# adityaX1412/Experiment-YOLO

Measured on AMD Instinct MI355X. Metric: images/sec (train) DEAL-YOLO-N 640x640 bs=64/GPU, higher is better.
Workload: dtype f16; 1 GPU; DEAL-YOLO-N (yolov8n-ASF-P2P2.yaml) train step 640x640, per-GPU batch 64, fwd+TAL/WIOU+NWD/DFL/BCE loss+bwd+SGD+EMA, BASELINE.json configs[1]; loss_mode=wiou+nwd, settle_steps=18, capture_retries=0, global_batch=64, parallelism=dp1, hipgraph=True

## Files before the change

### experiment-yolo_amd/csrc/conv_wgrad.hip

```cpp
#include <cstdio>
#include "common.h"
#include "dealyolo_hip.h"

typedef short short4v __attribute__((ext_vector_type(4)));
typedef unsigned int u32x4 __attribute__((ext_vector_type(4)));

struct WgArgs {
  const f16* x;
  const f16* dy;
  float* slabs;
  int ldx, lddy;
  int N, H, W, Ho, Wo;
  int cin_p, cout_p;
  int cin_r8, cout_r8;
  int nci_chunks;
  int tiles_x, tiles_y, ntiles;
  long npix;
  const f16* raw;
  f16* draw;
  const float* coef;
  const double* acc;
  float* dgamma;
  float* dbeta;
  int ldraw, cout;
  float count;
  DySegs xs;
  int dy_csplit;
  unsigned dy_plane;
  const f16* wt;
  f16* dx;
  int lddx, dx_acc;
  int dg_mt, dg_rows;
  DySegs dxs;
};

static __device__ __forceinline__ half8 tr_frag(const char* base0, const char* base1) {
  union {
    short4v s[2];
    half8 h;
  } u;
  u.s[0] = __builtin_amdgcn_ds_read_tr16_b64_v4i16((LDS_AS short4v*)(base0));
  u.s[1] = __builtin_amdgcn_ds_read_tr16_b64_v4i16((LDS_AS short4v*)(base1));
  return u.h;
}

static constexpr __host__ __device__ int wg_th(int ks, int stride, int nci, int mtc) {
  if (ks == 1) return (nci + mtc <= 4) ? 8 : 4;
  if (stride == 1) return (nci * mtc <= 1) ? 16 : ((nci + mtc <= 4) ? 8 : 4);
  return (nci * mtc <= 1) ? 8 : ((nci + mtc <= 4) ? 4 : 2);
}

template <int KS, int STRIDE, int NCI, int MTC, int BNF>
__global__ __launch_bounds__(256, (BNF & 8) ? 3 : ((KS == 3 && NCI * MTC >= 16) ? 1 : 2)) void conv_wgrad_kernel(const WgArgs a) {
  constexpr bool FLAT = (KS == 1);
  constexpr bool DG = (BNF & 4) != 0;
  constexpr bool NOX = (BNF & 8) != 0;
  static_assert(!NOX || DG, "the form without X exists for the fused input gradient only");
  constexpr bool BN1 = ((BNF & 3) == 1 || (BNF & 3) == 3);
  constexpr bool XSEG = ((BNF & 3) == 3);
  static_assert(!DG || (KS == 1 && BN1), "the fused input gradient exists for the 1x1 BatchNorm forms");
  constexpr int TAPS = KS * KS;
  constexpr int NCOL = NCI * TAPS;
  constexpr int CPW = (NCOL + 3) / 4;
  constexpr int TH = wg_th(KS, STRIDE, NCI, MTC), TW = 32;
  constexpr int HWX = FLAT ? TH * TW : (TW - 1) * STRIDE + KS;
  constexpr int HHX = FLAT ? 1 : (TH - 1) * STRIDE + KS;
  constexpr int PAD = KS / 2;
  constexpr int CIN_C = 16 * NCI, COUT_C = 16 * MTC;
  constexpr int PSX = (STRIDE == 2) ? CIN_C * 2 + 16 : (((CIN_C / 2 + 7) / 16) * 16 + 8) * 4;
  constexpr int PSY = (((COUT_C / 2 + 7) / 16) * 16 + 8) * 4;
  constexpr int XBYTES = NOX ? 0 : HHX * HWX * PSX, YBYTES = TH * TW * PSY;
  __shared__ __attribute__((aligned(16))) char smem[XBYTES + YBYTES];
  char* const sx = smem;
  char* const sy = smem + XBYTES;
  __shared__ __attribute__((aligned(16))) float sbn[BN1 ? 4 * COUT_C : (BNF == 2 ? 256 * 8 : 4)];
  float bsum[8] = {0.f, 0.f, 0.f, 0.f, 0.f, 0.f, 0.f, 0.f};
  (void)bsum;
  constexpr int DKS = MTC == 4 ? 2 : (MTC == 3 ? 3 : 1), DCPK = (MTC & 1) ? 16 : 32;
  constexpr int DNT = TH / 2;
  constexpr int DNC = 4 * NCI;
  constexpr int DXROW = CIN_C * 2 + 16;
  constexpr int DPPR = CIN_C / 8;
  constexpr int DPIXPASS = 64 / DPPR > 16 ? 16 : 64 / DPPR;
  constexpr int DNPASS = (16 + DPIXPASS - 1) / DPIXPASS;
  __shared__ __attribute__((aligned(16))) char sdx[DG ? 4 * 16 * DXROW : 16];

  const int tid = threadIdx.x, wave = tid >> 6, lane = tid & 63, p = lane & 15, q = lane >> 4;
  const int qq = p >> 2, pp = p & 3;
  const int co_chunk = blockIdx.y / a.nci_chunks, ci_chunk = blockIdx.y - co_chunk * a.nci_chunks;
  const int ci0 = ci_chunk * CIN_C, co0 = co_chunk * COUT_C;

  f32x4 acc[NOX ? 1 : MTC][NOX ? 1 : CPW];
  if (!NOX) {
#pragma unroll
    for (int m = 0; m < MTC; ++m)
#pragma unroll
      for (int c = 0; c < CPW; ++c) acc[NOX ? 0 : m][NOX ? 0 : c] = (f32x4){0.f, 0.f, 0.f, 0.f};
  }
  (void)acc;

  constexpr int NGX = HHX * HWX * (CIN_C / 8), NGY = TH * TW * (COUT_C / 8);
  constexpr int NPX = NOX ? 1 : (NGX + 255) / 256, NPY = (NGY + 255) / 256;
  uint4 pfx[NPX], pfy[NPY];
  uint4 pfr[BN1 ? NPY : 1];
  unsigned roff[BN1 ? NPY : 1];
  int ncur = 0, nnext = 0;
  (void)ncur; (void)nnext;
  unsigned vnext = 0, vcur = 0, ornext = 0, orcur = 0;
  (void)pfr; (void)roff; (void)vnext; (void)vcur; (void)ornext; (void)orcur;
  constexpr unsigned NEVER = 0x80000000u;
  constexpr int CPGX = CIN_C / 8, CPGY = COUT_C / 8;
  unsigned xoff[NPX], yoff[NPY];
  (void)pfx; (void)xoff;
#pragma unroll
  for (int i = 0; i < NPX; ++i) {
    const int id = tid + i * 256;
    const int pixel = id / CPGX, part = id - pixel * CPGX;
    const bool ok = !NOX && id < NGX && ci0 + part * 8 < a.cin_r8;
    const int hy = FLAT ? 0 : pixel / HWX, hx = FLAT ? pixel : pixel - hy * HWX;
    xoff[i] = ok ? (unsigned)(((hy * a.W + hx) * a.ldx + ci0 + part * 8) * 2) : NEVER;
  }
  constexpr bool XIN = XSEG && !NOX;
  const char* xb[XIN ? NPX : 1];
  int xl[XIN ? NPX : 1];
  unsigned xup = 0;
  bool any_up = false;
  if (XIN)
    for (int k = 0; k < a.xs.nseg; ++k) any_up = any_up || (a.xs.acc[k] & 2);
  (void)xb; (void)xl; (void)xup; (void)any_up;
  if (XIN) {
#pragma unroll
    for (int i = 0; i < NPX; ++i) {
      const int id = tid + i * 256;
      const int part = id % CPGX, ch = ci0 + part * 8;
      int sg = 0;
      while (sg + 1 < a.xs.nseg && ch >= a.xs.c_end[sg]) ++sg;
      const int cb = sg ? a.xs.c_end[sg - 1] : 0;
      const bool ok = id < NGX && ch < a.cin_r8;
      xb[XIN ? i : 0] = ok ? reinterpret_cast<const char*>(a.xs.ptr[sg]) + (ch - cb) * 2 : nullptr;
      xl[XIN ? i : 0] = a.xs.ld[sg] * 2;
      if (ok && (a.xs.acc[sg] & 2)) xup |= 1u << i;
    }
  }
#pragma unroll
  for (int i = 0; i < NPY; ++i) {
    const int id = tid + i * 256;
    const int pixel = id / CPGY, part = id - pixel * CPGY;
    const bool ok = id < NGY && co0 + part * 8 < a.cout_r8;
    const int ty = FLAT ? 0 : pixel / TW, tx = FLAT ? pixel : pixel - ty * TW;
    yoff[i] = ok ? (unsigned)(((ty * a.Wo + tx) * a.lddy + co0 + part * 8) * 2) : NEVER;
    if (FLAT && BN1 && a.dy_csplit && ok) {
      const int ch = co0 + part * 8;
      yoff[i] = (unsigned)((tx * a.lddy + (ch < a.dy_csplit ? ch : ch - a.dy_csplit)) * 2) + (ch < a.dy_csplit ? 0u : a.dy_plane);
    }
    if (BN1) roff[i] = ok ? (unsigned)(((ty * a.Wo + tx) * a.ldraw + co0 + part * 8) * 2) : NEVER;
  }
  if (BN1) {
    for (int c = tid; c < COUT_C; c += 256) {
      const int ch = co0 + c;
      float sc = 0.f, sh = 0.f, kb = 0.f, kc = 0.f;
// ... 24 lines not shown
  }
  half8 wf[DG ? DKS : 1][DG ? NCI : 1];
  unsigned dboff[DG ? DKS : 1];
  char* dxb = nullptr;
  unsigned dxld2 = 0;
  bool dxacc = false, dxadd = false;
  const int dpix = lane / DPPR, dpiece = lane - dpix * DPPR;
  (void)wf; (void)dboff; (void)dxb; (void)dxld2; (void)dxacc; (void)dxadd; (void)dpix; (void)dpiece;
  if (DG) {
#pragma unroll
    for (int k = 0; k < DKS; ++k) {
      dboff[DG ? k : 0] = (unsigned)((k * DCPK + ((q * 8) & (DCPK - 1))) * 2);
#pragma unroll
      for (int j = 0; j < NCI; ++j) {
        const int ch = ci0 + (p >> 2) * DNC + 4 * j + (p & 3);
        const int gw = 16 * a.dg_mt, g = ch / gw, rem = ch - g * gw;
        const int row = g * gw + ((rem % (4 * a.dg_mt)) >> 2) * 16 + (rem / (4 * a.dg_mt)) * 4 + (rem & 3);
        const int grow = (g * DKS + k) * gw + (row - g * gw);
        half8 v;
#pragma unroll
        for (int e = 0; e < 8; ++e) v[e] = (f16)0.f;
        if (row < a.dg_rows) v = *reinterpret_cast<const half8*>(a.wt + ((size_t)grow * 32 + q * 8));
        wf[DG ? k : 0][DG ? j : 0] = v;
      }
    }
    const int chn = ci0 + dpiece * 8;
    if (lane < DPIXPASS * DPPR && chn < a.cin_r8) {
      if (XSEG) {
        int sg = 0;
        while (sg + 1 < a.dxs.nseg && chn >= a.dxs.c_end[sg]) ++sg;
        const int cb = sg ? a.dxs.c_end[sg - 1] : 0;
        dxb = reinterpret_cast<char*>(const_cast<void*>(a.dxs.ptr[sg])) + (chn - cb) * 2;
        dxld2 = (unsigned)a.dxs.ld[sg] * 2u;
        dxacc = a.dxs.acc[sg] != 0;
      } else {
        dxb = reinterpret_cast<char*>(a.dx) + chn * 2;
        dxld2 = (unsigned)a.lddx * 2u;
        dxacc = a.dx_acc != 0;
      }
    }
    if (XSEG) {
      for (int k = 0; k < a.dxs.nseg; ++k) dxadd = dxadd || a.dxs.acc[k] != 0;
    } else {
      dxadd = a.dx_acc != 0;
    }
  }
  union DU4 { uint4 u; half2_ h[4]; };
  DU4 dold[DG ? DNT : 1][DG ? DNPASS : 1];
  (void)dold;
  auto ld16 = [](__amdgpu_buffer_rsrc_t r, unsigned off) {
    const auto v = __builtin_amdgcn_raw_buffer_load_b128(r, (int)off, 0, 0);
    return *reinterpret_cast<const uint4*>(&v);
  };
  auto prefetch = [&](int tile) {
    if (FLAT) {
      const auto rx = __builtin_amdgcn_make_buffer_rsrc(const_cast<f16*>(a.x), 0, (int)((unsigned)a.npix * (unsigned)a.ldx * 2u), 0x00020000);
      const auto ry = __builtin_amdgcn_make_buffer_rsrc(const_cast<f16*>(a.dy), 0, (int)((unsigned)a.npix * (unsigned)a.lddy * 2u + (a.dy_csplit ? a.dy_plane : 0u)), 0x00020000);
      const unsigned ox = (unsigned)tile * (TH * TW) * a.ldx * 2u, oy = (unsigned)tile * (TH * TW) * a.lddy * 2u;
      if (NOX) {
      } else if (XIN) {
        const long p0 = (long)tile * (TH * TW);
        int n0 = 0, y0 = 0, x0 = 0;
        if (any_up) {
          const int hw = a.H * a.W, g0 = (int)p0;
          n0 = g0 / hw;
          const int r0 = g0 - n0 * hw;
          y0 = r0 / a.W;
          x0 = r0 - y0 * a.W;
        }
        const float invW = 1.0f / (float)a.W, invH = 1.0f / (float)a.H;
#pragma unroll
        for (int i = 0; i < NPX; ++i) {
          const int lp = (tid + i * 256) / CPGX;
          long gp = p0 + lp;
          const bool inside = gp < a.npix;
          if ((xup >> i) & 1u) {
            const int xx = x0 + lp, dy_ = (int)(((float)xx + 0.5f) * invW), x = xx - dy_ * a.W;
            const int yt = y0 + dy_, dn = (int)(((float)yt + 0.5f) * invH), y = yt - dn * a.H;
            gp = ((long)(n0 + dn) * (a.H >> 1) + (y >> 1)) * (a.W >> 1) + (x >> 1);
          }
          const char* src = xb[XIN ? i : 0];
          pfx[i] = (src && inside) ? *reinterpret_cast<const uint4*>(src + gp * xl[XIN ? i : 0]) : make_uint4(0, 0, 0, 0);
        }
      } else {
#pragma unroll
        for (int i = 0; i < NPX; ++i) pfx[i] = ld16(rx, xoff[i] + ox);
      }
#pragma unroll
      for (int i = 0; i < NPY; ++i) pfy[i] = ld16(ry, yoff[i] + oy);
      if (BN1) {
        const unsigned nbytes = (unsigned)a.npix * (unsigned)a.ldraw * 2u;
        const auto rr = __builtin_amdgcn_make_buffer_rsrc(const_cast<f16*>(a.raw), 0, (int)nbytes, 0x00020000);
        ornext = (unsigned)tile * (TH * TW) * a.ldraw * 2u;
        vnext = 0;
#pragma unroll
        for (int i = 0; i < NPY; ++i) {
          const unsigned off = roff[i] + ornext;
          pfr[i] = ld16(rr, off);
          vnext |= (roff[i] != NEVER && off < nbytes) ? (1u << i) : 0u;
        }
      }
    } else {
      const int bx = tile % a.tiles_x;
      const int t2 = tile / a.tiles_x;
      const int n = t2 / a.tiles_y;
      const int oy0 = (t2 % a.tiles_y) * TH, ox0 = bx * TW;
      const int iy0 = oy0 * STRIDE - PAD, ix0 = ox0 * STRIDE - PAD;
      const auto rx = __builtin_amdgcn_make_buffer_rsrc(const_cast<f16*>(a.x) + (size_t)n * a.H * a.W * a.ldx, 0, a.H * a.W * a.ldx * 2, 0x00020000);
      const auto ry = __builtin_amdgcn_make_buffer_rsrc(const_cast<f16*>(a.dy) + (size_t)n * a.Ho * a.Wo * a.lddy, 0, a.Ho * a.Wo * a.lddy * 2, 0x00020000);
      const unsigned ox = (unsigned)((iy0 * a.W + ix0) * a.ldx * 2), oy = (unsigned)((oy0 * a.Wo + ox0) * a.lddy * 2);
      if (ix0 >= 0 && ix0 + HWX <= a.W) {
#pragma unroll
        for (int i = 0; i < NPX; ++i) pfx[i] = ld16(rx, xoff[i] + ox);
      } else {
#pragma unroll
        for (int i = 0; i < NPX; ++i) {
          const int hx = ((tid + i * 256) / CPGX) % HWX;
          pfx[i] = ld16(rx, (unsigned)(ix0 + hx) < (unsigned)a.W ? xoff[i] + ox : NEVER);
        }
      }
      if (ox0 + TW <= a.Wo) {
#pragma unroll
        for (int i = 0; i < NPY; ++i) pfy[i] = ld16(ry, yoff[i] + oy);
      } else {
#pragma unroll
        for (int i = 0; i < NPY; ++i) {
          const int tx = ((tid + i * 256) / CPGY) % TW;
          pfy[i] = ld16(ry, ox0 + tx < a.Wo ? yoff[i] + oy : NEVER);
        }
      }
      if (BN1) {
        const unsigned nbytes = (unsigned)(a.Ho * a.Wo * a.ldraw * 2);
        const auto rr = __builtin_amdgcn_make_buffer_rsrc(const_cast<f16*>(a.raw) + (size_t)n * a.Ho * a.Wo * a.ldraw, 0, (int)nbytes, 0x00020000);
        ornext = (unsigned)((oy0 * a.Wo + ox0) * a.ldraw * 2);
        vnext = 0;
        const bool xfull = ox0 + TW <= a.Wo;
#pragma unroll
        for (int i = 0; i < NPY; ++i) {
          unsigned off = roff[i] == NEVER ? NEVER : roff[i] + ornext;
          if (!xfull) {
            const int tx = ((tid + i * 256) / CPGY) % TW;
            off = ox0 + tx < a.Wo ? off : NEVER;
          }
          pfr[i] = ld16(rr, off);
          vnext |= off < nbytes ? (1u << i) : 0u;
        }
        nnext = n;
      }
    }
  };


  int tile = (!FLAT && !(gridDim.x & 7)) ? (int)(blockIdx.x & 7) * (int)(gridDim.x >> 3) + (int)(blockIdx.x >> 3) : (int)blockIdx.x;
  if (tile < a.ntiles) prefetch(tile);
  for (; tile < a.ntiles; tile += gridDim.x) {
    __syncthreads();
#pragma unroll
    for (int i = 0; i < NPX; ++i) {
      const int id = tid + i * 256;
      if (!NOX && id < NGX) *reinterpret_cast<uint4*>(sx + (id / (CIN_C / 8)) * PSX + (id % (CIN_C / 8)) * 16) = pfx[i];
    }
    if (BN1) {
      vcur = vnext; orcur = ornext; ncur = nnext;
      const unsigned nbytes = FLAT ? (unsigned)a.npix * (unsigned)a.ldraw * 2u : (unsigned)(a.Ho * a.Wo * a.ldraw * 2);
      const auto rd = __builtin_amdgcn_make_buffer_rsrc(FLAT ? a.draw : a.draw + (size_t)ncur * a.Ho * a.Wo * a.ldraw, 0, (int)nbytes, 0x00020000);
#pragma unroll
      for (int i = 0; i < NPY; ++i) {
        const int id = tid + i * 256;
        const int part = id % CPGY;
        const bool valid = (vcur >> i) & 1u;
        const float* cf = sbn + part * 8;
        union { half8 h; uint4 u; u32x4 v; } o;
        o.h = bn_bwd_apply8<DY_ACT_SILU>(*reinterpret_cast<const half8*>(&pfy[i]), *reinterpret_cast<const half8*>(&pfr[i]), cf,
                                         cf + COUT_C, cf + 2 * COUT_C, cf + 3 * COUT_C);
        if (!valid) o.u = make_uint4(0, 0, 0, 0);
        if (id < NGY) *reinterpret_cast<uint4*>(sy + (id / (COUT_C / 8)) * PSY + (id % (COUT_C / 8)) * 16) = o.u;
        if (!DG && ci_chunk == 0 && a.draw) __builtin_amdgcn_raw_buffer_store_b128(o.v, rd, (int)(valid ? roff[i] + orcur : NEVER), 0, 0);
      }
    } else {
#pragma unroll
      for (int i = 0; i < NPY; ++i) {
        const int id = tid + i * 256;
        if (id < NGY) *reinterpret_cast<uint4*>(sy + (id / (COUT_C / 8)) * PSY + (id % (COUT_C / 8)) * 16) = pfy[i];
        if (BNF == 2 && id < NGY) {
          const half8 v = *reinterpret_cast<const half8*>(&pfy[i]);
#pragma unroll
          for (int j = 0; j < 8; ++j) bsum[j] += (float)v[j];
        }
      }
    }
    __syncthreads();
    const long dpix0 = (long)tile * (TH * TW) + wave * (16 * DNT);
    (void)dpix0;
    if (DG && dxadd) {
#pragma unroll
      for (int t = 0; t < DNT; ++t)
#pragma unroll
        for (int ps = 0; ps < DNPASS; ++ps) {
          const int rowi = ps * DPIXPASS + dpix;
          const long gp = dpix0 + t * 16 + rowi;
          const bool ok = dxb && dxacc && rowi < 16 && gp < a.npix;
          dold[DG ? t : 0][DG ? ps : 0].u = ok ? *reinterpret_cast<const uint4*>(dxb + (size_t)gp * dxld2) : make_uint4(0, 0, 0, 0);
        }
      __builtin_amdgcn_sched_barrier(0);
    }
    if (tile + (int)gridDim.x < a.ntiles) prefetch(tile + gridDim.x);
// ... 193 lines not shown
    const int mid = (lo + hi + 1) >> 1;
    if (descs[mid].first_block <= (int)blockIdx.x) lo = mid;
    else hi = mid - 1;
  }
  const WgReduceDesc d = descs[lo];
  if (d.bias_c > 0 && (int)blockIdx.x == d.first_block && (int)threadIdx.x < d.bias_c) {
    double t = 0.0;
#pragma unroll
    for (int k = 0; k < DY_BN_COPIES; ++k) t += d.bias_acc[(size_t)k * d.bias_c + threadIdx.x];
    d.dbias[threadIdx.x] = (float)t;
  }
  wgrad_reduce_block(blockIdx.x - d.first_block, d.slabs, d.nslabs, d.dw, d.cout, d.cin, d.taps, d.cout_p, d.cin_p, d.accumulate,
                     d.ld_taps, d.ld_cphys, d.ld_cin);
}
extern "C" int dy_wgrad_reduce_desc_bytes(void) { return (int)sizeof(WgReduceDesc); }
static void wgrad_geometry(int cin, int cout, int ks, int stride, int* cin_p, int* cout_p, int* nci, int* mtc, long npix_out = 0);
extern "C" int dy_wgrad_reduce_desc_fill(void* desc, const float* slabs, int nslabs, float* dw, int cin, int cout, int ks, int stride,
                                         int accumulate, int ld_taps, int ld_cphys, int ld_cin, int first_block) {
  if (!desc || !slabs || !dw || nslabs < 1) return DY_ERR_ARG;
  int cp, op, nci, mtc;
  const int cin_eff = ld_taps ? ld_taps * ld_cphys : cin;
  wgrad_geometry(cin_eff, cout, ld_taps ? 1 : ks, ld_taps ? 1 : stride, &cp, &op, &nci, &mtc);
  const int taps = ld_taps ? 1 : ks * ks;
  WgReduceDesc* d = reinterpret_cast<WgReduceDesc*>(desc);
  *d = WgReduceDesc{slabs, dw, nslabs, cout, cin_eff, taps, op, cp, accumulate, ld_taps, ld_cphys, ld_cin, first_block, 0, nullptr, nullptr};
  return cdiv(taps * op * cp, 64);
}
extern "C" int dy_wgrad_reduce_desc_bias(void* desc, const double* bias_acc, float* dbias, int c) {
  if (!desc || !bias_acc || !dbias || c < 1 || c > 256) return DY_ERR_ARG;
  WgReduceDesc* d = reinterpret_cast<WgReduceDesc*>(desc);
  d->bias_acc = bias_acc; d->dbias = dbias; d->bias_c = c;
  return DY_OK;
}
extern "C" int dy_wgrad_reduce_batched(const void* descs_device, int n, int total_blocks, hipStream_t stream) {
  if (n <= 0 || total_blocks <= 0 || !descs_device) return DY_ERR_ARG;
  hipLaunchKernelGGL(wgrad_reduce_batched_kernel, dim3(total_blocks), dim3(256), 0, stream, (const WgReduceDesc*)descs_device, n);
  DY_CHECK_LAUNCH();
  return DY_OK;
}

template <int KS, int STRIDE, int NCI, int MTC>
static int launch_wgrad(const WgArgs& a, int gx, int gy, hipStream_t s) {
  if (a.wt) {
    if constexpr (KS == 1) {
      if (!a.raw || gy != a.nci_chunks) return DY_ERR_ARG;
      if (!a.x) {
        if (a.dxs.nseg > 0) hipLaunchKernelGGL((conv_wgrad_kernel<KS, STRIDE, NCI, MTC, 15>), dim3(gx, gy), dim3(256), 0, s, a);
        else hipLaunchKernelGGL((conv_wgrad_kernel<KS, STRIDE, NCI, MTC, 13>), dim3(gx, gy), dim3(256), 0, s, a);
      } else if (a.xs.nseg > 0) hipLaunchKernelGGL((conv_wgrad_kernel<KS, STRIDE, NCI, MTC, 7>), dim3(gx, gy), dim3(256), 0, s, a);
      else hipLaunchKernelGGL((conv_wgrad_kernel<KS, STRIDE, NCI, MTC, 5>), dim3(gx, gy), dim3(256), 0, s, a);
    } else return DY_ERR_ARG;
  } else if (a.raw && a.xs.nseg > 0) {
    if constexpr (KS == 1) hipLaunchKernelGGL((conv_wgrad_kernel<KS, STRIDE, NCI, MTC, 3>), dim3(gx, gy), dim3(256), 0, s, a);
    else return DY_ERR_ARG;
  } else if (a.raw) hipLaunchKernelGGL((conv_wgrad_kernel<KS, STRIDE, NCI, MTC, 1>), dim3(gx, gy), dim3(256), 0, s, a);
  else if (a.acc && MTC != 3) hipLaunchKernelGGL((conv_wgrad_kernel<KS, STRIDE, NCI, MTC, 2>), dim3(gx, gy), dim3(256), 0, s, a);
  else if (a.acc) return DY_ERR_ARG;
  else hipLaunchKernelGGL((conv_wgrad_kernel<KS, STRIDE, NCI, MTC, 0>), dim3(gx, gy), dim3(256), 0, s, a);
  DY_CHECK_LAUNCH();
  return DY_OK;
}
template <int KS, int STRIDE>
static int dispatch_wgrad(int nci, int mtc, const WgArgs& a, int gx, int gy, hipStream_t s) {
#define DY_CASE(I, M) \
  if (nci == I && mtc == M) return launch_wgrad<KS, STRIDE, I, M>(a, gx, gy, s);
  DY_CASE(1, 1) DY_CASE(1, 2) DY_CASE(1, 4)
  DY_CASE(2, 1) DY_CASE(2, 2) DY_CASE(2, 4)
  if (!(KS == 3 && STRIDE == 2)) { DY_CASE(4, 1) DY_CASE(4, 2) DY_CASE(4, 4) }
  if (KS == 1) {
    DY_CASE(3, 1) DY_CASE(3, 2) DY_CASE(3, 4) DY_CASE(1, 3) DY_CASE(2, 3) DY_CASE(4, 3) DY_CASE(3, 3)
  }
#undef DY_CASE
  return DY_ERR_ARG;
}

static int wgrad_per_cu(int ks, int nci, int mtc) {
  static const int light = getenv("DY_WGRAD_LIGHT_WGS") ? atoi(getenv("DY_WGRAD_LIGHT_WGS")) : 2;
  if (ks == 3 && nci * mtc >= 16) return 1;
  return nci * mtc <= 2 ? light : 2;
}
static long wgrad_columns(int ks, int nci, int mtc, int cp, int op) {
  const int gy = (cp / (16 * nci)) * (op / (16 * mtc));
  const int per_cu = wgrad_per_cu(ks, nci, mtc);
  int gx = (256 * per_cu) / gy;
  return gx < 32 ? 32 : gx;
}
static void wgrad_geometry(int cin, int cout, int ks, int stride, int* cin_p, int* cout_p, int* nci, int* mtc, long npix_out) {
  *cin_p = (cin + 15) / 16 * 16;
  *cout_p = (cout + 15) / 16 * 16;
  const int cit = *cin_p / 16, cot = *cout_p / 16;
  const int cap = (ks == 3 && stride == 2) ? 2 : 4;
  *nci = (cit % 4 == 0 && cap >= 4) ? 4 : ((ks == 1 && cit % 3 == 0) ? 3 : (cit % 2 == 0 ? 2 : 1));
  *mtc = cot % 4 == 0 ? 4 : ((ks == 1 && cot % 3 == 0) ? 3 : (cot % 2 == 0 ? 2 : 1));
  static const bool split = !(getenv("DY_WGRAD_SPLIT") && atoi(getenv("DY_WGRAD_SPLIT")) == 0);
  static const double f = getenv("DY_WGRAD_SPLIT_F") ? atof(getenv("DY_WGRAD_SPLIT_F")) : 2.0;
  if (!split || npix_out <= 0) return;
  const double wbytes = (double)ks * ks * *cin_p * *cout_p * 4.0;
  const double act = (double)npix_out * (*cin_p * stride * stride + *cout_p) * 2.0;
  while (2.0 * wgrad_columns(ks, *nci, *mtc, *cin_p, *cout_p) * wbytes > f * act) {
    if (*mtc % 2 == 0 && *mtc >= *nci) *mtc /= 2;
    else if (*nci % 2 == 0) *nci /= 2;
    else if (*mtc % 2 == 0) *mtc /= 2;
    else break;
  }
}

extern "C" int dy_wgrad_workspace(int n, int h, int w, int cin, int cout, int ks, int stride, int* nslabs,
                                  long* slab_elems) {
  int cp, op, nci, mtc;
  const int pad = ks / 2, Ho = (h + 2 * pad - ks) / stride + 1, Wo = (w + 2 * pad - ks) / stride + 1;
  wgrad_geometry(cin, cout, ks, stride, &cp, &op, &nci, &mtc, (long)n * Ho * Wo);
  const int th = wg_th(ks, stride, nci, mtc);
  int ntiles;
  if (ks == 1) ntiles = (int)(((long)n * Ho * Wo + th * 32 - 1) / (th * 32));
  else ntiles = cdiv(Wo, 32) * cdiv(Ho, th) * n;
  *slab_elems = (long)ks * ks * cp * op;
  const int gy = (cp / (16 * nci)) * (op / (16 * mtc));
  const int per_cu = wgrad_per_cu(ks, nci, mtc);
  int gx = (256 * per_cu) / gy;
  if (gx < 32) gx = 32;
  static const int tpb = getenv("DY_WGRAD_TPB") ? atoi(getenv("DY_WGRAD_TPB")) : 1;
  if (tpb > 1 && gx > ntiles / tpb) gx = ntiles / tpb > 32 ? ntiles / tpb : (ntiles < 32 ? ntiles : 32);
  if (gx > ntiles) gx = ntiles;
  if (gx < 1) gx = 1;
  *nslabs = gx;
  return DY_OK;
}

struct WgBnHost {
  const void* raw; void* draw; const float* coef; const double* acc; float* dgamma; float* dbeta; int ldraw; float count;
  const DySegs* xs = nullptr;
  int dy_csplit = 0;
  unsigned dy_plane = 0;
  const void* wt = nullptr; void* dx = nullptr; int lddx = 0, dx_acc = 0; const DySegs* dxs = nullptr;
  bool dgrad_only = false;
};
static int conv_wgrad_impl(const void* x, int ldx, const void* dy, int lddy, float* slabs, float* dw, int n, int h, int w,
                           int cin, int cout, int ks, int stride, int accumulate, int ld_taps, int ld_cphys, int ld_cin,
                           hipStream_t stream, const WgBnHost* bn = nullptr);

extern "C" int dy_wgrad_kernel_name(int cin, int cout, int ks, int stride, char* out, int cap) {
  if (!out || cap < 8) return DY_ERR_ARG;
  int cp, op, nci, mtc;
  wgrad_geometry(cin, cout, ks, stride, &cp, &op, &nci, &mtc);
  snprintf(out, cap, "conv_wgrad_kernel<%d, %d, %d, %d, 0>", ks, stride, nci, mtc);
  return DY_OK;
}

extern "C" int dy_wgrad_kernel_name_at(int n, int h, int w, int cin, int cout, int ks, int stride, char* out, int cap) {
  if (!out || cap < 8) return DY_ERR_ARG;
  int cp, op, nci, mtc;
  wgrad_geometry(cin, cout, ks, stride, &cp, &op, &nci, &mtc,
                 (long)n * ((h + 2 * (ks / 2) - ks) / stride + 1) * ((w + 2 * (ks / 2) - ks) / stride + 1));
  snprintf(out, cap, "conv_wgrad_kernel<%d, %d, %d, %d, 0>", ks, stride, nci, mtc);
  return DY_OK;
}

extern "C" int dy_conv_wgrad(const void* x, int ldx, const void* dy, int lddy, float* slabs, float* dw, int n, int h,
                             int w, int cin, int cout, int ks, int stride, int accumulate, hipStream_t stream) {
  return conv_wgrad_impl(x, ldx, dy, lddy, slabs, dw, n, h, w, cin, cout, ks, stride, accumulate, 0, 0, 0, stream);
}
extern "C" int dy_conv_wgrad_ld(const void* x, int ldx, const void* dy, int lddy, float* slabs, float* dw, int n, int h,
                                int w, int cout, int ld_cin, int ld_taps, int ld_cphys, int accumulate, hipStream_t stream) {
  return conv_wgrad_impl(x, ldx, dy, lddy, slabs, dw, n, h, w, ld_taps * ld_cphys, cout, 1, 1, accumulate, ld_taps, ld_cphys,
                         ld_cin, stream);
}

extern "C" int dy_conv_wgrad_bn(const void* x, int ldx, const void* dy, int lddy, const void* raw, int ldraw, void* draw,
                                const float* coef, const double* acc, float* dgamma, float* dbeta, float count, float* slabs,
                                float* dw, int n, int h, int w, int cin, int cout, int ks, int stride, int accumulate,
                                hipStream_t stream) {
  if (!raw || !coef || !acc || (ldraw & 7) || ((uintptr_t)raw & 15) || ((uintptr_t)draw & 15) || (cout & 15)) return DY_ERR_ARG;
  const WgBnHost bn{raw, draw, coef, acc, dgamma, dbeta, ldraw, count};
  return conv_wgrad_impl(x, ldx, dy, lddy, slabs, dw, n, h, w, cin, cout, ks, stride, accumulate, 0, 0, 0, stream, &bn);
}
extern "C" int dy_conv_wgrad_bias(const void* x, int ldx, const void* dy, int lddy, double* bias_acc, float* slabs, float* dw, int n,
                                  int h, int w, int cin, int cout, int ks, int stride, int accumulate, hipStream_t stream) {
  if (!bias_acc) return DY_ERR_ARG;
  const WgBnHost bn{nullptr, nullptr, nullptr, bias_acc, nullptr, nullptr, 0, 1.f};
  return conv_wgrad_impl(x, ldx, dy, lddy, slabs, dw, n, h, w, cin, cout, ks, stride, accumulate, 0, 0, 0, stream, &bn);
}
extern "C" int dy_conv1x1_wgrad_bn_segs(const DySegs* xs, const void* dy, int lddy, const void* raw, int ldraw, void* draw, const float* coef,
                                        const double* acc, float* dgamma, float* dbeta, float count, float* slabs, float* dw, int n, int h,
                                        int w, int cin, int cout, int accumulate, hipStream_t stream) {
  if (!raw || !coef || !acc || (ldraw & 7) || ((uintptr_t)raw & 15) || ((uintptr_t)draw & 15) || (cout & 15)) return DY_ERR_ARG;
  if (!xs || xs->nseg < 1 || xs->nseg > DY_MAX_SEGS || xs->c_end[xs->nseg - 1] != cin) return DY_ERR_ARG;
  for (int k = 0; k < xs->nseg; ++k)
    if ((xs->c_end[k] & 7) || (xs->ld[k] & 7) || !xs->ptr[k] || ((uintptr_t)xs->ptr[k] & 15) || xs->c_end[k] <= (k ? xs->c_end[k - 1] : 0) ||
        ((xs->acc[k] & 2) && ((h | w) & 1))) return DY_ERR_ARG;
  WgBnHost bn{raw, draw, coef, acc, dgamma, dbeta, ldraw, count};
  bn.xs = xs;
  return conv_wgrad_impl(xs->ptr[0], 8, dy, lddy, slabs, dw, n, h, w, cin, cout, 1, 1, accumulate, 0, 0, 0, stream, &bn);
}
extern "C" int dy_conv1x1_wgrad_bn_planes(const DySegs* xs, const void* x, int ldx, const void* dy, const void* dy2, int lddy, int csplit,
                                          const void* raw, int ldraw, void* draw, const float* coef, const double* acc, float* dgamma,
                                          float* dbeta, float count, float* slabs, float* dw, int n, int h, int w, int cin, int cout,
                                          int accumulate, hipStream_t stream) {
  if (!raw || !coef || !acc || (ldraw & 7) || ((uintptr_t)raw & 15) || ((uintptr_t)draw & 15) || (cout & 15)) return DY_ERR_ARG;
  if (!dy || !dy2 || (csplit & 7) || csplit <= 0 || csplit >= cout || ((uintptr_t)dy2 & 15)) return DY_ERR_ARG;
  const long plane = (const char*)dy2 - (const char*)dy;
  if (plane < (long)n * h * w * lddy * 2 || plane + (double)n * h * w * lddy * 2.0 >= 2147483648.0) return DY_ERR_ARG;
  if (xs) {
    if (xs->nseg < 1 || xs->nseg > DY_MAX_SEGS || xs->c_end[xs->nseg - 1] != cin) return DY_ERR_ARG;
    for (int k = 0; k < xs->nseg; ++k)
      if ((xs->c_end[k] & 7) || (xs->ld[k] & 7) || !xs->ptr[k] || ((uintptr_t)xs->ptr[k] & 15) || xs->c_end[k] <= (k ? xs->c_end[k - 1] : 0) ||
          ((xs->acc[k] & 2) && ((h | w) & 1))) return DY_ERR_ARG;
  }
  WgBnHost bn{raw, draw, coef, acc, dgamma, dbeta, ldraw, count};
  bn.xs = xs;
  bn.dy_csplit = csplit; bn.dy_plane = (unsigned)plane;
  return conv_wgrad_impl(xs ? xs->ptr[0] : x, xs ? 8 : ldx, dy, lddy, slabs, dw, n, h, w, cin, cout, 1, 1, accumulate, 0, 0, 0, stream, &bn);
}

struct WgDgPlan { int ok, nci, mtc, dg_mt, dg_rows; };
static WgDgPlan wgrad_dgrad_plan(int n, int h, int w, int cin, int cout) {
  WgDgPlan r{};
  if (n < 1 || h < 1 || w < 1 || cin < 8 || (cin & 7) || cout < 16 || (cout & 15) || cout > 64) return r;
  int cp, op, nci, mtc;
  wgrad_geometry(cin, cout, 1, 1, &cp, &op, &nci, &mtc, (long)n * h * w);
  if (16 * mtc != op) return r;
  int gcin, gcout, cc, nch, mt, ng, kst, pe;
  if (dy_conv_geometry(cout, cin, 1, 1, &gcin, &gcout, &cc, &nch, &mt, &ng, &kst, &pe) != DY_OK) return r;
  const int dks = mtc == 4 ? 2 : (mtc == 3 ? 3 : 1), dcpk = (mtc & 1) ? 16 : 32;
  if (gcin != cout || nch * kst != dks || (cc < 32 ? cc : 32) != dcpk || gcout < cp) return r;
  r.ok = 1; r.nci = nci; r.mtc = mtc; r.dg_mt = mt; r.dg_rows = gcout;
  return r;
// ... 91 lines not shown
                                                int lddx, int dx_accumulate, const DySegs* dxs, int n, int h, int w, int cin, int cout,
                                                int accumulate, hipStream_t stream) {
  if (!raw || !coef || !acc || (ldraw & 7) || ((uintptr_t)raw & 15)) return DY_ERR_ARG;
  if (!dy || !dy2 || (csplit & 7) || csplit <= 0 || csplit >= cout || ((uintptr_t)dy2 & 15)) return DY_ERR_ARG;
  const long plane = (const char*)dy2 - (const char*)dy;
  if (plane < (long)n * h * w * lddy * 2 || plane + (double)n * h * w * lddy * 2.0 >= 2147483648.0) return DY_ERR_ARG;
  if (!w_packed_t || ((uintptr_t)w_packed_t & 15) || !wgrad_dgrad_plan(n, h, w, cin, cout).ok) return DY_ERR_ARG;
  if (xs) {
    if (!segs_in_valid(xs, cin, h, w) || !dgrad_segs_valid(xs, dxs)) return DY_ERR_ARG;
  } else if (dxs || !dx || ((uintptr_t)dx & 15) || (lddx & 7) || lddx < cin || (double)n * h * w * lddx * 2.0 >= 2147483648.0) {
    return DY_ERR_ARG;
  }
  WgBnHost bn{raw, nullptr, coef, acc, dgamma, dbeta, ldraw, count};
  bn.xs = xs; bn.dy_csplit = csplit; bn.dy_plane = (unsigned)plane;
  bn.wt = w_packed_t; bn.dxs = xs ? dxs : nullptr; bn.dx = xs ? nullptr : dx; bn.lddx = lddx; bn.dx_acc = dx_accumulate != 0;
  return conv_wgrad_impl(xs ? xs->ptr[0] : x, xs ? 8 : ldx, dy, lddy, slabs, dw, n, h, w, cin, cout, 1, 1, accumulate, 0, 0, 0, stream, &bn);
}
extern "C" int dy_conv_wgrad_ld_bn(const void* x, int ldx, const void* dy, int lddy, const void* raw, int ldraw, void* draw,
                                   const float* coef, const double* acc, float* dgamma, float* dbeta, float count, float* slabs,
                                   float* dw, int n, int h, int w, int cout, int ld_cin, int ld_taps, int ld_cphys, int accumulate,
                                   hipStream_t stream) {
  if (!raw || !coef || !acc || (ldraw & 7) || ((uintptr_t)raw & 15) || ((uintptr_t)draw & 15) || (cout & 15)) return DY_ERR_ARG;
  const WgBnHost bn{raw, draw, coef, acc, dgamma, dbeta, ldraw, count};
  return conv_wgrad_impl(x, ldx, dy, lddy, slabs, dw, n, h, w, ld_taps * ld_cphys, cout, 1, 1, accumulate, ld_taps, ld_cphys, ld_cin,
                         stream, &bn);
}

static int conv_wgrad_impl(const void* x, int ldx, const void* dy, int lddy, float* slabs, float* dw, int n, int h, int w,
                           int cin, int cout, int ks, int stride, int accumulate, int ld_taps, int ld_cphys, int ld_cin,
                           hipStream_t stream, const WgBnHost* bn) {
  if (!(ks == 1 || ks == 3) || !(stride == 1 || stride == 2) || (ks == 1 && stride != 1)) return DY_ERR_ARG;
  if ((ldx & 7) || (lddy & 7) || ((uintptr_t)x & 15) || ((uintptr_t)dy & 15)) return DY_ERR_ALIGN;
  const bool dgrad_only = bn && bn->dgrad_only;
  if (dgrad_only != (x == nullptr) || (dgrad_only && (!bn->wt || slabs || dw))) return DY_ERR_ARG;
  if ((ks == 1 ? (double)n : 1.0) * h * w * (ldx > lddy ? ldx : lddy) * 2.0 >= 2147483648.0) return DY_ERR_ARG;
  int cp, op, nci, mtc;
  wgrad_geometry(cin, cout, ks, stride, &cp, &op, &nci, &mtc,
                 (long)n * ((h + 2 * (ks / 2) - ks) / stride + 1) * ((w + 2 * (ks / 2) - ks) / stride + 1));
  WgArgs a{};
  a.x = (const f16*)x; a.dy = (const f16*)dy; a.slabs = slabs; a.ldx = ldx; a.lddy = lddy;
  a.N = n; a.H = h; a.W = w;
  const int pad = ks / 2;
  a.Ho = (h + 2 * pad - ks) / stride + 1;
  a.Wo = (w + 2 * pad - ks) / stride + 1;
  a.cin_p = cp; a.cout_p = op;
  a.cin_r8 = (cin + 7) / 8 * 8; a.cout_r8 = (cout + 7) / 8 * 8;
  if (bn) {
    if ((ks == 1 ? (double)n : 1.0) * a.Ho * a.Wo * bn->ldraw * 2.0 >= 2147483648.0) return DY_ERR_ARG;
    a.raw = (const f16*)bn->raw; a.draw = (f16*)bn->draw; a.coef = bn->coef; a.acc = bn->acc;
    a.dgamma = bn->dgamma; a.dbeta = bn->dbeta; a.ldraw = bn->ldraw; a.count = bn->count;
    a.cout = bn->raw ? cout : (cout + 7) / 8 * 8;
    if (bn->xs) a.xs = *bn->xs;
    a.dy_csplit = bn->dy_csplit; a.dy_plane = bn->dy_plane;
    if (bn->wt) {
      const WgDgPlan pl = wgrad_dgrad_plan(n, h, w, cin, cout);
      if (!pl.ok || pl.nci != nci || pl.mtc != mtc || ks != 1 || ld_taps) return DY_ERR_ARG;
      a.wt = (const f16*)bn->wt; a.dx = (f16*)bn->dx; a.lddx = bn->lddx; a.dx_acc = bn->dx_acc;
      a.dg_mt = pl.dg_mt; a.dg_rows = pl.dg_rows;
      if (bn->dxs) a.dxs = *bn->dxs;
    }
  }
  a.nci_chunks = cp / (16 * nci);
  const int nco_chunks = op / (16 * mtc);
  const int th = wg_th(ks, stride, nci, mtc);
  if (ks == 1) {
    a.npix = (long)n * a.Ho * a.Wo;
    a.ntiles = (int)((a.npix + th * 32 - 1) / (th * 32));
  } else {
    a.tiles_x = cdiv(a.Wo, 32);
    a.tiles_y = cdiv(a.Ho, th);
    a.ntiles = a.tiles_x * a.tiles_y * n;
  }
  int nslabs;
  long slab_elems;
  dy_wgrad_workspace(n, h, w, cin, cout, ks, stride, &nslabs, &slab_elems);
  const int gy = a.nci_chunks * nco_chunks;
  if (dgrad_only) nslabs = dgrad_only_columns(a.ntiles, gy);
  int rc;
  if (ks == 1) rc = dispatch_wgrad<1, 1>(nci, mtc, a, nslabs, gy, stream);
  else if (stride == 1) rc = dispatch_wgrad<3, 1>(nci, mtc, a, nslabs, gy, stream);
  else rc = dispatch_wgrad<3, 2>(nci, mtc, a, nslabs, gy, stream);
  if (rc != DY_OK) return rc;
  if (!dw) return DY_OK;
  const int total = ks * ks * op * cp;
  hipLaunchKernelGGL(wgrad_reduce_kernel, dim3(cdiv(total, 64)), dim3(256), 0, stream, slabs, nslabs, dw, cout, cin,
                     ks * ks, op, cp, accumulate, ld_taps, ld_cphys, ld_cin);
  DY_CHECK_LAUNCH();
  return DY_OK;
}
```

### experiment-yolo_amd/csrc/head_rows.hip

```cpp
#include <hip/hip_runtime.h>

#include <cstdlib>

#include "common.h"
#include "dealyolo_hip.h"

template <typename T>
struct Levels {
  int nl;
  T lv[4];
};
struct RowsArgs {
  const f16* x;
  const f16* dy;
  const int* flag;
  const float* w;
  f16* dx;
  float* slabs;
  double* bias_acc;
  int ldx, lddy, lddx, A, a0, hw, B, dx_acc;
  const float* xcoef;
  int nblk, dgx;
};

// ... 25 lines not shown
          fl[k] = a.flag[(size_t)b * a.A + a.a0 + r];
        }
      }
    }
    int mine = -1;
#pragma unroll
    for (int k = 0; k < FB; ++k)
      if ((trip & (FB - 1)) == k) mine = fl[k];
    const bool fg = mine >= 0;
    const unsigned long long m = __ballot(fg);
    if (lane == 0) s_cnt[wave] = __popcll(m);
    __syncthreads();
    int base = 0, total = 0;
#pragma unroll
    for (int w = 0; w < 4; ++w) {
      if (w < wave) base += s_cnt[w];
      total += s_cnt[w];
    }
    if (fg) s_list[base + __popcll(m & ((1ull << lane) - 1ull))] = tid;
    __syncthreads();
    for (int i0 = 0; i0 < total; i0 += 16) {
      const int nb = total - i0 < 16 ? total - i0 : 16;
      {
        const int i = tid >> 4, g = tid & 15;
        if (i < nb) {
          const long q = p0 + s_list[i0 + i];
          if (g < 8) {
            half8 xv = *reinterpret_cast<const half8*>(a.x + q * a.ldx + g * 8);
            if (a.xcoef) xv = bn_silu_apply8(xv, a.xcoef + g * 8, a.xcoef + 64 + g * 8);
            *reinterpret_cast<half8*>(s_x + i * 64 + g * 8) = xv;
          } else {
            *reinterpret_cast<uint4*>(s_dy + i * 64 + (g - 8) * 8) = *reinterpret_cast<const uint4*>(a.dy + q * a.lddy + (g - 8) * 8);
          }
        }
      }
      __syncthreads();
      for (int i = 0; i < nb; ++i) {
        const float g = (float)s_dy[i * 64 + co];
#pragma unroll
        for (int k = 0; k < 16; ++k) acc[k] += g * (float)s_x[i * 64 + ci0 + k];
        if ((tid & 3) == 0) bs += g;
      }
      __syncthreads();
    }
  }
  float* slab = a.slabs + (size_t)blockIdx.x * 64 * 64 + co * 64 + ci0;
#pragma unroll
  for (int k = 0; k < 16; k += 4) *reinterpret_cast<float4*>(slab + k) = make_float4(acc[k], acc[k + 1], acc[k + 2], acc[k + 3]);
  if ((tid & 3) == 0 && bs != 0.f) unsafeAtomicAdd(a.bias_acc + (size_t)(blockIdx.x % DY_BN_COPIES) * 64 + co, (double)bs);
}

__global__ __launch_bounds__(256) void rows_dgrad_kernel(Levels<RowsArgs> L) {
  const RowsArgs& a = L.lv[blockIdx.z];
  if (!a.dx || (int)blockIdx.x >= a.dgx || (int)blockIdx.y >= a.B) return;
  __shared__ float s_w[64 * 65];
  for (int i = threadIdx.x; i < 64 * 64; i += 256) s_w[(i >> 6) * 65 + (i & 63)] = (float)(f16)a.w[i];
  __syncthreads();
  const int b = blockIdx.y, part = threadIdx.x & 7, ci0 = part * 8;
  const int* const fl = a.flag + (size_t)b * a.A + a.a0;
  for (int r = (int)(blockIdx.x * 32 + (threadIdx.x >> 3)); r < a.hw; r += a.dgx * 32) {
    const long p = (long)b * a.hw + r;
    f16* const dst = a.dx + p * a.lddx + ci0;
    if (fl[r] < 0) {
      if (!a.dx_acc) *reinterpret_cast<uint4*>(dst) = make_uint4(0, 0, 0, 0);
      continue;
    }
    float s[8];
#pragma unroll
    for (int k = 0; k < 8; ++k) s[k] = 0.f;
    const f16* const g = a.dy + p * a.lddy;
    for (int c8 = 0; c8 < 64; c8 += 8) {
      const half8 gv = *reinterpret_cast<const half8*>(g + c8);
#pragma unroll
      for (int j = 0; j < 8; ++j) {
        const float gg = (float)gv[j];
#pragma unroll
        for (int k = 0; k < 8; ++k) s[k] += gg * s_w[(c8 + j) * 65 + ci0 + k];
      }
    }
    half8 o;
    if (a.dx_acc) {
      const half8 old = *reinterpret_cast<const half8*>(dst);
#pragma unroll
      for (int k = 0; k < 8; ++k) o[k] = (f16)((float)old[k] + s[k]);
    } else {
#pragma unroll
      for (int k = 0; k < 8; ++k) o[k] = (f16)s[k];
    }
    *reinterpret_cast<half8*>(dst) = o;
  }
}

static __device__ __forceinline__ float exp_nonpos(float x) {
  const float t = x * 1.44269502f;
  float r = __builtin_fmaf(x, 1.44269502f, -t);
  r = __builtin_fmaf(x, 1.92596299e-8f, r);
  const float e = __builtin_amdgcn_exp2f(t);
  return __builtin_fmaf(e, r * 0.693147182f, e);
}
static __device__ __forceinline__ f32x2 exp_nonpos2(f32x2 x) {
  const f32x2 l2e = {1.44269502f, 1.44269502f}, l2e_lo = {1.92596299e-8f, 1.92596299e-8f}, ln2 = {0.693147182f, 0.693147182f};
  const f32x2 t = x * l2e;
  f32x2 r = __builtin_elementwise_fma(x, l2e, -t);
  r = __builtin_elementwise_fma(x, l2e_lo, r);
  const f32x2 e = {__builtin_amdgcn_exp2f(t[0]), __builtin_amdgcn_exp2f(t[1])};
  return __builtin_elementwise_fma(e, r * ln2, e);
}
struct BoxDecArgs {
  const f16* x;
  const float* w;
  const float* bias;
  float* pred_box;
  int ldx, A, a0, hw, W, B;
  const float* xcoef;
  int nblk;
};
template <bool LIBM>
__global__ __launch_bounds__(256) void head_box_decode_kernel(Levels<BoxDecArgs> L) {
  const BoxDecArgs& a = L.lv[blockIdx.y];
  if ((int)blockIdx.x >= a.nblk) return;
  auto ex = [](float x) { return LIBM ? expf(x) : exp_nonpos(x); };
  constexpr int PITCH = 160;
  __shared__ __attribute__((aligned(16))) char s_w[64 * PITCH];
  __shared__ float s_b[64];
  const int tid = threadIdx.x, wave = tid >> 6, lane = tid & 63, p = lane & 15, q = lane >> 4;
  for (int i = tid; i < 64 * 64; i += 256) {
    const int c = i >> 6, k = i & 63;
    const int row = ((c >> 2) & 3) * 16 + (c >> 4) * 4 + (c & 3);
    *reinterpret_cast<f16*>(s_w + row * PITCH + k * 2) = (f16)a.w[i];
  }
  if (tid < 64) s_b[tid] = a.bias[tid];
  __syncthreads();
  const long npix = (long)a.B * a.hw;
  const float invw = 1.0f / (float)a.W;
  float csc[2][8], csh[2][8];
  if (a.xcoef) {
#pragma unroll
    for (int ks = 0; ks < 2; ++ks)
#pragma unroll
      for (int j = 0; j < 8; ++j) {
        csc[ks][j] = a.xcoef[ks * 32 + q * 8 + j];
        csh[ks][j] = a.xcoef[64 + ks * 32 + q * 8 + j];
// ... 62 lines not shown
      const float anc = (q & 1) ? (iy + 0.5f) : (ix + 0.5f);
      a.pred_box[((size_t)b * a.A + a.a0 + r) * 4 + q] = q < 2 ? anc - e : anc + e;
    }
  }
}
static int box_decode_fill(BoxDecArgs& a, const void* x, int ldx, const float* x_coef, const float* weight, const float* bias, float* pred_box,
                           int A, int a0, int n, int h, int w, int cin, int cout) {
  if (cin != 64 || cout != 64 || !x || !weight || !bias || !pred_box || n < 1 || h < 1 || w < 1 || a0 < 0 || a0 + h * w > A) return DY_ERR_ARG;
  if ((ldx & 7) || ((uintptr_t)x & 15)) return DY_ERR_ALIGN;
  static const int cap = getenv("DY_HEAD_DECODE_WGS") ? atoi(getenv("DY_HEAD_DECODE_WGS")) : 2048;
  long blocks = ((long)n * h * w + 255) / 256;
  if (blocks > cap) blocks = cap;
  a = BoxDecArgs{(const f16*)x, weight, bias, pred_box, ldx, A, a0, h * w, w, n, x_coef, (int)blocks};
  return DY_OK;
}
static int box_decode_launch(const Levels<BoxDecArgs>& L, hipStream_t stream) {
  int gx = 1;
  for (int l = 0; l < L.nl; ++l) gx = L.lv[l].nblk > gx ? L.lv[l].nblk : gx;
  static const bool libm = getenv("DY_DECODE_LIBM_EXP") && atoi(getenv("DY_DECODE_LIBM_EXP")) != 0;
  if (libm) hipLaunchKernelGGL(head_box_decode_kernel<true>, dim3(gx, L.nl), dim3(256), 0, stream, L);
  else hipLaunchKernelGGL(head_box_decode_kernel<false>, dim3(gx, L.nl), dim3(256), 0, stream, L);
  DY_CHECK_LAUNCH();
  return DY_OK;
}
extern "C" int dy_head_box_decode(const void* x, int ldx, const float* x_coef, const float* weight, const float* bias, float* pred_box, int A,
                                  int a0, int n, int h, int w, int cin, int cout, hipStream_t stream) {
  Levels<BoxDecArgs> L{};
  L.nl = 1;
  const int rc = box_decode_fill(L.lv[0], x, ldx, x_coef, weight, bias, pred_box, A, a0, n, h, w, cin, cout);
  return rc != DY_OK ? rc : box_decode_launch(L, stream);
}
extern "C" int dy_head_box_decode_levels(int nl, const void* const* x, const int* ldx, const float* const* x_coef, const float* const* weight,
                                         const float* const* bias, float* pred_box, int A, const int* a0, int n, const int* h, const int* w,
                                         int cin, int cout, hipStream_t stream) {
  if (nl < 1 || nl > 4) return DY_ERR_ARG;
  Levels<BoxDecArgs> L{};
  L.nl = nl;
  for (int l = 0; l < nl; ++l) {
    const int rc = box_decode_fill(L.lv[l], x[l], ldx[l], x_coef ? x_coef[l] : nullptr, weight[l], bias[l], pred_box, A, a0[l], n, h[l], w[l], cin, cout);
    if (rc != DY_OK) return rc;
  }
  return box_decode_launch(L, stream);
}

extern "C" int dy_conv1x1_rows_supported(int cin, int cout) { return cin == 64 && cout == 64; }
extern "C" int dy_conv1x1_rows_slabs(int n, int h, int w) {
  const long ns = (long)n * h * w / 2048;
  return ns < 64 ? 64 : (ns > 1024 ? 1024 : (int)ns);
}
static int rows_fill(RowsArgs& a, const void* x, int ldx, const float* x_coef, const void* dy, int lddy, const int* assigned, int A, int a0,
                     const float* weight, void* dx, int lddx, int dx_accumulate, float* slabs, double* bias_acc, int n, int h, int w, int cin,
                     int cout) {
  if (!dy_conv1x1_rows_supported(cin, cout) || !x || !dy || !assigned || !weight || !slabs || !bias_acc || n < 1 || h < 1 || w < 1 ||
      a0 < 0 || a0 + h * w > A)
    return DY_ERR_ARG;
  if ((ldx & 7) || (lddy & 7) || (dx && (lddx & 7)) || ((uintptr_t)x & 15) || ((uintptr_t)dy & 15) || ((uintptr_t)dx & 15) ||
      ((uintptr_t)slabs & 15))
    return DY_ERR_ALIGN;
  int gx = (h * w + 1023) / 1024;
  if (gx > 16) gx = 16;
  a = RowsArgs{(const f16*)x, (const f16*)dy, assigned, weight, (f16*)dx, slabs, bias_acc, ldx, lddy, lddx, A, a0, h * w, n, dx_accumulate, x_coef,
               dy_conv1x1_rows_slabs(n, h, w), gx};
  return DY_OK;
}
static int rows_launch(const Levels<RowsArgs>& L, hipStream_t stream) {
  int gw = 1, gd = 0, nb = 1;
  for (int l = 0; l < L.nl; ++l) {
    gw = L.lv[l].nblk > gw ? L.lv[l].nblk : gw;
    if (L.lv[l].dx) gd = L.lv[l].dgx > gd ? L.lv[l].dgx : gd;
    nb = L.lv[l].B > nb ? L.lv[l].B : nb;
  }
  hipLaunchKernelGGL(rows_wgrad_kernel, dim3(gw, L.nl), dim3(256), 0, stream, L);
  if (gd) hipLaunchKernelGGL(rows_dgrad_kernel, dim3(gd, nb, L.nl), dim3(256), 0, stream, L);
  DY_CHECK_LAUNCH();
  return DY_OK;
}
extern "C" int dy_conv1x1_rows_backward(const void* x, int ldx, const float* x_coef, const void* dy, int lddy, const int* assigned, int A, int a0,
                                        const float* weight, void* dx, int lddx, int dx_accumulate, float* slabs, double* bias_acc,
                                        int n, int h, int w, int cin, int cout, hipStream_t stream) {
  Levels<RowsArgs> L{};
  L.nl = 1;
  const int rc = rows_fill(L.lv[0], x, ldx, x_coef, dy, lddy, assigned, A, a0, weight, dx, lddx, dx_accumulate, slabs, bias_acc, n, h, w, cin, cout);
  return rc != DY_OK ? rc : rows_launch(L, stream);
}
extern "C" int dy_conv1x1_rows_backward_levels(int nl, const void* const* x, const int* ldx, const float* const* x_coef, const void* const* dy,
                                               const int* lddy, const int* assigned, int A, const int* a0, const float* const* weight,
                                               void* const* dx, const int* lddx, const int* dx_accumulate, float* const* slabs,
                                               double* const* bias_acc, int n, const int* h, const int* w, int cin, int cout,
                                               hipStream_t stream) {
  if (nl < 1 || nl > 4) return DY_ERR_ARG;
  Levels<RowsArgs> L{};
  L.nl = nl;
  for (int l = 0; l < nl; ++l) {
    const int rc = rows_fill(L.lv[l], x[l], ldx[l], x_coef ? x_coef[l] : nullptr, dy[l], lddy[l], assigned, A, a0[l], weight[l], dx[l], lddx[l],
                             dx_accumulate[l], slabs[l], bias_acc[l], n, h[l], w[l], cin, cout);
    if (rc != DY_OK) return rc;
  }
  return rows_launch(L, stream);
}

struct ClsArgs {
  const f16* x;
  const float* xcoef;
  const float* w;
  const float* bias;
  float* y;
  const f16* dy;
  f16* dx;
  float* slabs;
  double* bias_acc;
  int ldx, lddx, nc, dx_acc;
  long npix;
  int nblk;
};
template <int CIN>
__global__ __launch_bounds__(256) void cls_head_fwd_kernel(Levels<ClsArgs> L) {
  const ClsArgs& a = L.lv[blockIdx.y];
  if ((int)blockIdx.x >= a.nblk) return;
  constexpr int PARTS = CIN / 8, PPB = 256 / PARTS;
  __shared__ float s_w[8][CIN], s_b[8];
  for (int i = threadIdx.x; i < 8 * CIN; i += 256) s_w[i / CIN][i % CIN] = (i / CIN) < a.nc ? (float)(f16)a.w[i] : 0.f;
  if (threadIdx.x < 8) s_b[threadIdx.x] = threadIdx.x < a.nc ? a.bias[threadIdx.x] : 0.f;
  __syncthreads();
  const int part = threadIdx.x % PARTS, k0 = part * 8;
  float sc[8], sh[8];
  if (a.xcoef) {
#pragma unroll
    for (int j = 0; j < 8; ++j) { sc[j] = a.xcoef[k0 + j]; sh[j] = a.xcoef[CIN + k0 + j]; }
  }
  for (long pix = (long)blockIdx.x * PPB + threadIdx.x / PARTS; pix < a.npix; pix += (long)a.nblk * PPB) {
    half8 xv = *reinterpret_cast<const half8*>(a.x + pix * a.ldx + k0);
    if (a.xcoef) xv = bn_silu_apply8(xv, sc, sh);
    float o[8];
#pragma unroll
    for (int c = 0; c < 8; ++c) {
      float t = 0.f;
#pragma unroll
      for (int j = 0; j < 8; ++j) t += s_w[c][k0 + j] * (float)xv[j];
      o[c] = t;
    }
#pragma unroll
    for (int c = 0; c < 8; ++c) o[c] = PARTS == 4 ? quad_sum(o[c]) : half_row_sum(o[c]);
    if (part == 0) {
      float* dst = a.y + pix * 8;
      *reinterpret_cast<float4*>(dst) = make_float4(o[0] + s_b[0], o[1] + s_b[1], o[2] + s_b[2], o[3] + s_b[3]);
      *reinterpret_cast<float4*>(dst + 4) = make_float4(o[4] + s_b[4], o[5] + s_b[5], o[6] + s_b[6], o[7] + s_b[7]);
    }
  }
}
template <int CIN>
__global__ __launch_bounds__(256) void cls_head_bwd_kernel(Levels<ClsArgs> L) {
  const ClsArgs& a = L.lv[blockIdx.y];
  if ((int)blockIdx.x >= a.nblk) return;
  constexpr int PARTS = CIN / 8, PPB = 256 / PARTS;
  __shared__ float s_w[8][CIN];
  __shared__ float s_red[4][PARTS][64];
  __shared__ float s_bs[4][8];
  for (int i = threadIdx.x; i < 8 * CIN; i += 256) s_w[i / CIN][i % CIN] = (i / CIN) < a.nc ? (float)(f16)a.w[i] : 0.f;
  __syncthreads();
  const int tid = threadIdx.x, wave = tid >> 6, lane = tid & 63, part = tid % PARTS, k0 = part * 8;
  float sc[8], sh[8];
  if (a.xcoef) {
#pragma unroll
    for (int j = 0; j < 8; ++j) { sc[j] = a.xcoef[k0 + j]; sh[j] = a.xcoef[CIN + k0 + j]; }
  }
  float acc[8][8], bs[8];
#pragma unroll
  for (int c = 0; c < 8; ++c) {
    bs[c] = 0.f;
#pragma unroll
    for (int j = 0; j < 8; ++j) acc[c][j] = 0.f;
  }
  const long chunk = ((a.npix + a.nblk - 1) / a.nblk + PPB - 1) / PPB * PPB;
  const long lo = (long)blockIdx.x * chunk, hi = lo + chunk < a.npix ? lo + chunk : a.npix;
  for (long pix = lo + tid / PARTS; pix < hi; pix += PPB) {
    half8 xv = *reinterpret_cast<const half8*>(a.x + pix * a.ldx + k0);
    const half8 dv = *reinterpret_cast<const half8*>(a.dy + pix * 8);
    if (a.xcoef) xv = bn_silu_apply8(xv, sc, sh);
    float d[8], g[8];
#pragma unroll
    for (int c = 0; c < 8; ++c) d[c] = (float)dv[c];
#pragma unroll
    for (int j = 0; j < 8; ++j) g[j] = 0.f;
#pragma unroll
    for (int c = 0; c < 8; ++c) {
#pragma unroll
      for (int j = 0; j < 8; ++j) {
        acc[c][j] += d[c] * (float)xv[j];
        g[j] += s_w[c][k0 + j] * d[c];
      }
      if (part == 0) bs[c] += d[c];
    }
    if (a.dx) {
      f16* dst = a.dx + pix * a.lddx + k0;
      half8 o;
      if (a.dx_acc) {
        const half8 old = *reinterpret_cast<const half8*>(dst);
#pragma unroll
        for (int j = 0; j < 8; ++j) o[j] = (f16)((float)old[j] + g[j]);
      } else {
#pragma unroll
        for (int j = 0; j < 8; ++j) o[j] = (f16)g[j];
      }
      *reinterpret_cast<half8*>(dst) = o;
    }
  }
#pragma unroll
  for (int c = 0; c < 8; ++c) {
#pragma unroll
    for (int j = 0; j < 8; ++j) {
      float v = acc[c][j];
#pragma unroll
      for (int m = PARTS; m < 64; m <<= 1) v += __shfl_xor(v, m, 64);
      acc[c][j] = v;
    }
    float b = bs[c];
#pragma unroll
    for (int m = PARTS; m < 64; m <<= 1) b += __shfl_xor(b, m, 64);
    bs[c] = b;
  }
  if (lane < PARTS) {
#pragma unroll
    for (int c = 0; c < 8; ++c)
#pragma unroll
      for (int j = 0; j < 8; ++j) s_red[wave][lane][c * 8 + j] = acc[c][j];
  }
  if (lane == 0) {
#pragma unroll
    for (int c = 0; c < 8; ++c) s_bs[wave][c] = bs[c];
  }
  __syncthreads();
  float* slab = a.slabs + (size_t)blockIdx.x * 16 * CIN;
  for (int i = tid; i < 16 * CIN; i += 256) {
    const int co = i / CIN, ci = i - co * CIN;
    float v = 0.f;
    if (co < 8) {
      const int pp = ci >> 3, j = ci & 7;
      v = (s_red[0][pp][co * 8 + j] + s_red[1][pp][co * 8 + j]) + (s_red[2][pp][co * 8 + j] + s_red[3][pp][co * 8 + j]);
    }
    slab[i] = v;
  }
  if (tid < 8) {
    const float b = (s_bs[0][tid] + s_bs[1][tid]) + (s_bs[2][tid] + s_bs[3][tid]);
    if (b != 0.f) unsafeAtomicAdd(a.bias_acc + (size_t)(blockIdx.x % DY_BN_COPIES) * 8 + tid, (double)b);
  }
}
extern "C" int dy_cls_head_supported(int cin, int nc) { return (cin == 32 || cin == 64) && nc >= 1 && nc <= 8; }
extern "C" int dy_cls_head_slabs(void) { return 512; }
static int cls_fill(ClsArgs& a, bool backward, const void* x, int ldx, const float* x_coef, const float* weight, const float* bias, float* logits,
                    const void* dy, void* dx, int lddx, int dx_accumulate, float* slabs, double* bias_acc, long npix, int cin, int nc) {
  if (!dy_cls_head_supported(cin, nc) || !x || !weight || npix < 1) return DY_ERR_ARG;
  if (!backward && (!bias || !logits)) return DY_ERR_ARG;
  if (backward && (!dy || !slabs || !bias_acc)) return DY_ERR_ARG;
  if ((ldx & 7) || (dx && (lddx & 7)) || ((uintptr_t)x & 15) || ((uintptr_t)logits & 15) || ((uintptr_t)dy & 15) || ((uintptr_t)dx & 15))
    return DY_ERR_ALIGN;
  int nblk;
  if (backward) {
    nblk = dy_cls_head_slabs();
  } else {
    const int ppb = 256 / (cin / 8);
    long blocks = (npix + ppb - 1) / ppb;
    nblk = (int)(blocks > 4096 ? 4096 : blocks);
  }
  a = ClsArgs{(const f16*)x, x_coef, weight, bias, logits, (const f16*)dy, (f16*)dx, slabs, bias_acc, ldx, lddx, nc, dx_accumulate, npix, nblk};
  return DY_OK;
}
static int cls_launch(const Levels<ClsArgs>& L, bool backward, int cin, hipStream_t stream) {
  int gx = 1;
  for (int l = 0; l < L.nl; ++l) gx = L.lv[l].nblk > gx ? L.lv[l].nblk : gx;
  const dim3 grid(gx, L.nl);
  if (!backward && cin == 32) hipLaunchKernelGGL(cls_head_fwd_kernel<32>, grid, dim3(256), 0, stream, L);
  else if (!backward) hipLaunchKernelGGL(cls_head_fwd_kernel<64>, grid, dim3(256), 0, stream, L);
  else if (cin == 32) hipLaunchKernelGGL(cls_head_bwd_kernel<32>, grid, dim3(256), 0, stream, L);
  else hipLaunchKernelGGL(cls_head_bwd_kernel<64>, grid, dim3(256), 0, stream, L);
  DY_CHECK_LAUNCH();
  return DY_OK;
}
extern "C" int dy_cls_head_forward(const void* x, int ldx, const float* x_coef, const float* weight, const float* bias, float* logits,
                                   long npix, int cin, int nc, hipStream_t stream) {
  Levels<ClsArgs> L{};
  L.nl = 1;
  const int rc = cls_fill(L.lv[0], false, x, ldx, x_coef, weight, bias, logits, nullptr, nullptr, 0, 0, nullptr, nullptr, npix, cin, nc);
  return rc != DY_OK ? rc : cls_launch(L, false, cin, stream);
}
extern "C" int dy_cls_head_backward(const void* x, int ldx, const float* x_coef, const void* dy, const float* weight, void* dx, int lddx,
                                    int dx_accumulate, float* slabs, double* bias_acc, long npix, int cin, int nc, hipStream_t stream) {
  Levels<ClsArgs> L{};
  L.nl = 1;
  const int rc = cls_fill(L.lv[0], true, x, ldx, x_coef, weight, nullptr, nullptr, dy, dx, lddx, dx_accumulate, slabs, bias_acc, npix, cin, nc);
  return rc != DY_OK ? rc : cls_launch(L, true, cin, stream);
}
extern "C" int dy_cls_head_forward_levels(int nl, const void* const* x, const int* ldx, const float* const* x_coef, const float* const* weight,
                                          const float* const* bias, float* const* logits, const long* npix, int cin, int nc,
                                          hipStream_t stream) {
  if (nl < 1 || nl > 4) return DY_ERR_ARG;
  Levels<ClsArgs> L{};
  L.nl = nl;
  for (int l = 0; l < nl; ++l) {
    const int rc = cls_fill(L.lv[l], false, x[l], ldx[l], x_coef ? x_coef[l] : nullptr, weight[l], bias[l], logits[l], nullptr, nullptr, 0, 0, nullptr,
                            nullptr, npix[l], cin, nc);
    if (rc != DY_OK) return rc;
  }
  return cls_launch(L, false, cin, stream);
}
extern "C" int dy_cls_head_backward_levels(int nl, const void* const* x, const int* ldx, const float* const* x_coef, const void* const* dy,
                                           const float* const* weight, void* const* dx, const int* lddx, const int* dx_accumulate,
                                           float* const* slabs, double* const* bias_acc, const long* npix, int cin, int nc,
                                           hipStream_t stream) {
  if (nl < 1 || nl > 4) return DY_ERR_ARG;
  Levels<ClsArgs> L{};
  L.nl = nl;
  for (int l = 0; l < nl; ++l) {
    const int rc = cls_fill(L.lv[l], true, x[l], ldx[l], x_coef ? x_coef[l] : nullptr, weight[l], nullptr, nullptr, dy[l], dx[l], lddx[l],
                            dx_accumulate[l], slabs[l], bias_acc[l], npix[l], cin, nc);
    if (rc != DY_OK) return rc;
  }
  return cls_launch(L, true, cin, stream);
}
```

### experiment-yolo_amd/csrc/loss.hip

```cpp
#include "common.h"
#include "dealyolo_hip.h"

#define REG_MAX 16
#define TOPK 10
#define TAL_EPS 1e-9f
#define IOU_EPS 1e-7f

struct Level {
  const float* box;
  const float* cls;
  f16* dbox;
  f16* dcls;
  int H, W, a0;
  float stride;
  const f16* xin = nullptr;
  int ldin = 0;
  const float* w = nullptr;
  const float* bias = nullptr;
  const float* incoef = nullptr;
};
struct BoxMode {
  int family, ltype, fm, modifier;
  float inner_ratio, focaler_d, focaler_u, shape_scale, piou_lambda;
  float mpd_hw_num;
// ... 297 lines not shown
  const Dual cw = dmaximum(x2, dconst(t[2])) - dminimum(x1, dconst(t[0]));
  const Dual ch = dmaximum(y2, dconst(t[3])) - dminimum(y1, dconst(t[1]));
  if (m.ltype == DY_BOX_GIOU) {
    const Dual ca = cw * ch + IOU_EPS;
    return I - (ca - uni) / ca;
  }
  const Dual c2 = (dsq(cw) + dsq(ch)) + IOU_EPS;
  const Dual sx = ((t[0] + t[2]) - x1) - x2, sy = ((t[1] + t[3]) - y1) - y2;
  const Dual rho2 = (dsq(sx) + dsq(sy)) / 4.f;
  switch (m.ltype) {
    case DY_BOX_CIOU: {
      const Dual v = (float)(4.0 / (M_PI * M_PI)) * dsq(atanf(w2 / h2) - t_atan(w1 / h1));
      const float alpha = v.v / ((v.v - Ia.v) + (1.f + IOU_EPS));
      return I - (rho2 / c2 + v * alpha);
    }
    case DY_BOX_EIOU: {
      const Dual rw2 = dsq((t[2] - t[0]) - (x2 - x1)), rh2 = dsq((t[3] - t[1]) - (y2 - y1));
      return I - ((rho2 / c2 + rw2 / (dsq(cw) + IOU_EPS)) + rh2 / (dsq(ch) + IOU_EPS));
    }
    case DY_BOX_SIOU: {
      const Dual scw = sx * 0.5f + IOU_EPS, sch = sy * 0.5f + IOU_EPS;
      const Dual sigma = t_sqrt(dsq(scw) + dsq(sch));
      const Dual s1 = dabs(scw) / sigma, s2 = dabs(sch) / sigma;
      const Dual sa = dsel(s1.v > 0.70710678118654752f, s2, s1);
      const Dual gamma = dcos(dasin(sa) * 2.f - (float)(M_PI / 2)) - 2.f;
      const Dual dc = (2.f - t_exp(gamma * dsq(scw / cw))) - t_exp(gamma * dsq(sch / ch));
      const Dual ow = dabs(w1 - w2) / dmaximum(w1, dconst(w2)), oh = dabs(h1 - h2) / dmaximum(h1, dconst(h2));
      const Dual sc = dpow4(1.f - t_exp(-ow)) + dpow4(1.f - t_exp(-oh));
      return (I - 0.5f * (dc + sc)) + IOU_EPS;
    }
    case DY_BOX_SHAPEIOU: {
      const float pws = powf(w2, m.shape_scale), phs = powf(h2, m.shape_scale);
      const float ww = 2.f * pws / (pws + phs), hh = 2.f * phs / (pws + phs);
      const Dual dist = (hh * (dsq(sx) / 4.f) + ww * (dsq(sy) / 4.f)) / c2;
      const Dual ow = (hh * dabs(w1 - w2)) / dmaximum(w1, dconst(w2)), oh = (ww * dabs(h1 - h2)) / dmaximum(h1, dconst(h2));
      const Dual sc = dpow4(1.f - t_exp(-ow)) + dpow4(1.f - t_exp(-oh));
      return (I - dist) - 0.5f * sc;
    }
    case DY_BOX_PIOU:
    case DY_BOX_PIOU2: {
      const Dual dw1 = dabs(dminimum(x2, x1) - fminf(t[2], t[0])), dw2 = dabs(dmaximum(x2, x1) - fmaxf(t[2], t[0]));
      const Dual dh1 = dabs(dminimum(y2, y1) - fminf(t[3], t[1])), dh2 = dabs(dmaximum(y2, y1) - fmaxf(t[3], t[1]));
      const Dual P = ((dw1 + dw2) / fabsf(w2) + (dh1 + dh2) / fabsf(h2)) / 4.f;
      const Dual pv1 = ((1.f - I) - t_exp(-dsq(P))) + 1.f;
      if (m.ltype == DY_BOX_PIOU) return 1.f - pv1;
      const Dual x = t_exp(-P) * m.piou_lambda;
      return 1.f - ((3.f * x) * t_exp(-dsq(x))) * pv1;
    }
    default:
      return I - rho2 / c2;
  }
}

__global__ void pack_targets_kernel(LossCtx c, const float* bidx, const float* cls, const float* boxes, int n,
                                    const int* n_dev, float img_w, float img_h) {
  if (n_dev) n = *n_dev;
  for (int i = blockIdx.x * blockDim.x + threadIdx.x; i < c.B * c.nmax; i += gridDim.x * blockDim.x) {
    c.gt_valid[i] = 0;
    c.gt_cls[i] = 0;
    c.pos_align[i] = 0u;
    c.pos_ov[i] = 0u;
    for (int k = 0; k < 4; ++k) c.gt_box[i * 4 + k] = 0.f;
  }
  if (threadIdx.x == 0) c.scal[9] = 0.f;
  __shared__ short sb[8192];
  const int ncache = n < 8192 ? n : 8192;
  for (int i = threadIdx.x; i < ncache; i += blockDim.x) sb[i] = (short)(int)bidx[i];
  __syncthreads();
  for (int i = threadIdx.x; i < n; i += blockDim.x) {
    const int b = (int)bidx[i];
    if (b < 0 || b >= c.B) continue;
    int slot = 0;
    for (int j = 0; j < i; ++j) slot += ((j < ncache ? (int)sb[j] : (int)bidx[j]) == b);
    if (slot >= c.nmax) {
      c.scal[9] = 1.f;
      c.scal[10] = 1.f;
      continue;
    }
    const float x = boxes[i * 4 + 0] * img_w, y = boxes[i * 4 + 1] * img_h;
    const float w = boxes[i * 4 + 2] * img_w, h = boxes[i * 4 + 3] * img_h;
    const float dw = w / 2, dh = h / 2;
    float* g = c.gt_box + ((size_t)b * c.nmax + slot) * 4;
    g[0] = x - dw; g[1] = y - dh; g[2] = x + dw; g[3] = y + dh;
    c.gt_cls[b * c.nmax + slot] = (int)cls[i];
    c.gt_valid[b * c.nmax + slot] = (g[0] + g[1] + g[2] + g[3]) > 0.f ? 1 : 0;
  }
}

static __device__ __forceinline__ float softmax16_expect(float logit, int bin, float& prob) {
  float m = logit;
  m = fmaxf(m, __shfl_xor(m, 1, 64));
  m = fmaxf(m, __shfl_xor(m, 2, 64));
  m = fmaxf(m, __shfl_xor(m, 4, 64));
  m = fmaxf(m, __shfl_xor(m, 8, 64));
  const float e = expf(logit - m);
  const float s = quad16_sum(e);
  prob = e / s;
  return quad16_sum(prob * (float)bin);
}

__global__ __launch_bounds__(256) void decode_kernel(LossCtx c) {
  const int sub = threadIdx.x & 15, side = sub >> 2, quarter = sub & 3;
  const int b = blockIdx.y;
  float invw[4];
#pragma unroll
  for (int k = 0; k < 4; ++k) invw[k] = k < c.nl ? 1.0f / (float)c.lv[k].W : 0.f;
  for (int a = (int)((blockIdx.x * 256 + threadIdx.x) >> 4); a < c.A; a += (int)((gridDim.x * 256) >> 4)) {
    int l = 0;
#pragma unroll
    for (int k = 1; k < 4; ++k)
      if (k < c.nl && a >= c.lv[k].a0) l = k;
    const Level& L = c.lv[l];
    const int r = a - L.a0;
    const int iy = (int)(((float)r + 0.5f) * invw[l]), ix = r - iy * L.W;
    const float4 v = *reinterpret_cast<const float4*>(L.box + ((size_t)b * (L.H * L.W) + r) * 64 + sub * 4);
    float m = fmaxf(fmaxf(v.x, v.y), fmaxf(v.z, v.w));
    m = fmaxf(m, __shfl_xor(m, 1, 64));
    m = fmaxf(m, __shfl_xor(m, 2, 64));
    const float e0 = expf(v.x - m), e1 = expf(v.y - m), e2 = expf(v.z - m), e3 = expf(v.w - m);
    float den = (e0 + e1) + (e2 + e3);
    const float k0 = (float)(quarter * 4);
    float num = e0 * k0 + e1 * (k0 + 1.f) + e2 * (k0 + 2.f) + e3 * (k0 + 3.f);
    den += __shfl_xor(den, 1, 64);
    num += __shfl_xor(num, 1, 64);
    den += __shfl_xor(den, 2, 64);
    num += __shfl_xor(num, 2, 64);
// ... 514 lines not shown
  hipLaunchKernelGGL(tal_scatter_kernel, dim3(cdiv((int)BN * TOPK, 256)), dim3(256), 0, stream, c);
  const int gridE = (int)((BA + 255) / 256 < 2048 ? (BA + 255) / 256 : 2048);
  hipLaunchKernelGGL(tal_resolve_kernel, dim3(gridE), dim3(256), 0, stream, c);
  hipLaunchKernelGGL(tal_scores_kernel, dim3(gridE), dim3(256), 0, stream, c);
  DY_CHECK_LAUNCH();
  return DY_OK;
}

extern "C" int dy_loss_args_bytes(void) { return (int)sizeof(DyLossArgs); }
extern "C" int dy_detection_loss(const DyLossArgs* d, hipStream_t stream) {
  if (d->nl < 1 || d->nl > 4 || d->nmax < 1 || (d->ncp & 7) || d->nc > d->ncp) return DY_ERR_ARG;
  LossCtx c{};
  c.nl = d->nl; c.B = d->B; c.nc = d->nc; c.ncp = d->ncp; c.nmax = d->nmax;
  int a0 = 0;
  for (int l = 0; l < d->nl; ++l) {
    c.lv[l] = Level{d->box[l], d->cls[l], (f16*)d->dbox[l], (f16*)d->dcls[l], d->H[l], d->W[l], a0, d->stride[l]};
    if (d->box_from_input) {
      if (!d->box_in[l] || !d->box_w[l] || !d->box_b[l] || (d->box_in_ld[l] & 7)) return DY_ERR_ARG;
      c.lv[l].box = nullptr;
      c.lv[l].xin = (const f16*)d->box_in[l]; c.lv[l].ldin = d->box_in_ld[l]; c.lv[l].w = d->box_w[l]; c.lv[l].bias = d->box_b[l];
      c.lv[l].incoef = d->box_in_coef[l];
    }
    a0 += d->H[l] * d->W[l];
  }
  c.A = a0;
  char* p = (char*)d->workspace;
  auto take = [&](size_t b) { char* r = p; p += (b + 255) / 256 * 256; return r; };
  const size_t BA = (size_t)c.B * c.A, BN = (size_t)c.B * c.nmax;
  c.gt_box = (float*)take(BN * 16); c.gt_cls = (int*)take(BN * 4); c.gt_valid = (int*)take(BN * 4);
  c.pred_box = (float*)take(BA * 16); c.cnt = (int*)take(BA * 4); c.owner = (int*)take(BA * 4);
  c.asg_gt = (int*)take(BA * 4); c.asg_metric = (float*)take(BA * 4); c.asg_ov = (float*)take(BA * 4);
  c.tscore = (float*)take(BA * 4);
  c.topk_idx = (int*)take(BN * TOPK * 4); c.pos_align = (unsigned*)take(BN * 4); c.pos_ov = (unsigned*)take(BN * 4);
  float* scal_ws = (float*)take(16 * 4);
  (void)scal_ws;
  c.scal = d->scalars;
  float* partA = (float*)take(3 * 4096 * 4);
  float* partB = (float*)take(2 * 4096 * 4);
  float* partC = (float*)take(4 * 4096 * 4);
  c.hyp_box = d->hyp_box; c.hyp_cls = d->hyp_cls; c.hyp_dfl = d->hyp_dfl;
  c.use_wiou = d->use_wiou; c.use_nwd = d->use_nwd; c.iou_ratio = d->iou_ratio; c.gscale = d->gscale;
  if (d->box_family != DY_BOX_FAMILY_LEGACY) {
    const int fam = d->box_family, lt = d->box_ltype, mod = d->box_modifier;
    if (fam != DY_BOX_FAMILY_WISE && fam != DY_BOX_FAMILY_BBOX) return DY_ERR_ARG;
    if (lt < DY_BOX_IOU || lt > DY_BOX_MPDIOU || (fam == DY_BOX_FAMILY_BBOX && lt == DY_BOX_WIOU)) return DY_ERR_ARG;
    if (mod < DY_BOX_MOD_PLAIN || mod > DY_BOX_MOD_FOCALER) return DY_ERR_ARG;
    if (fam == DY_BOX_FAMILY_WISE && (d->box_fm < DY_BOX_FM_V1 || d->box_fm > DY_BOX_FM_V3)) return DY_ERR_ARG;
    if (mod == DY_BOX_MOD_FOCALER && !(d->focaler_u != d->focaler_d)) return DY_ERR_ARG;
    c.bm = BoxMode{fam, lt, d->box_fm, mod, d->inner_ratio, d->focaler_d, d->focaler_u, d->shape_scale, d->piou_lambda,
                   d->img_h * d->img_h + d->img_w * d->img_w};
    c.use_wiou = fam == DY_BOX_FAMILY_WISE;
  }

  hipLaunchKernelGGL(pack_targets_kernel, dim3(1), dim3(1024), 0, stream, c, d->t_batch_idx, d->t_cls, d->t_boxes,
                     d->n_targets, d->n_targets_dev, d->img_w, d->img_h);
  if (hipMemsetAsync(c.cnt, 0, BA * 4, stream) != hipSuccess) return DY_ERR_LAUNCH;
  const int gridA = (int)((BA * 64 + 255) / 256 < 2048 ? (BA * 64 + 255) / 256 : 2048);
  if (!d->box_from_input) {
    const long nb = ((long)c.A * 16 + 255) / 256;
    hipLaunchKernelGGL(decode_kernel, dim3((int)(nb < 256 ? nb : 256), c.B), dim3(256), 0, stream, c);
  }
  hipLaunchKernelGGL(tal_topk_kernel, dim3((int)BN), dim3(256), 0, stream, c);
  hipLaunchKernelGGL(tal_scatter_kernel, dim3(cdiv((int)BN * TOPK, 256)), dim3(256), 0, stream, c);
  const int gridE = (int)((BA + 255) / 256 < 2048 ? (BA + 255) / 256 : 2048);
  hipLaunchKernelGGL(tal_resolve_kernel, dim3(gridE), dim3(256), 0, stream, c);
  c.partials = partA;
  hipLaunchKernelGGL(tal_scores_kernel, dim3(gridE), dim3(256), 0, stream, c);
  hipLaunchKernelGGL(loss_scalars_kernel, dim3(1), dim3(256), 0, stream, c, gridE);
  int n_cls = 0;
  for (int l = 0; l < c.nl; ++l) {
    const long tot = (long)c.B * c.lv[l].H * c.lv[l].W;
    int g = (int)((tot + 255) / 256 < 2048 ? (tot + 255) / 256 : 2048);
    c.partials = partC + n_cls;
    hipLaunchKernelGGL(cls_loss_kernel, dim3(g), dim3(256), 0, stream, c, l);
    n_cls += g;
  }
  c.partials = partB;
  for (int l = 0; l < c.nl; ++l)
    if (c.lv[l].dbox && !d->dbox_rows_only && hipMemsetAsync(c.lv[l].dbox, 0, (size_t)c.B * c.lv[l].H * c.lv[l].W * 64 * 2, stream) != hipSuccess)
      return DY_ERR_LAUNCH;
  if (c.bm.family != DY_BOX_FAMILY_LEGACY)
    hipLaunchKernelGGL(box_loss_kernel<true>, dim3(gridA), dim3(256), 0, stream, c);
  else
    hipLaunchKernelGGL(box_loss_kernel<false>, dim3(gridA), dim3(256), 0, stream, c);
  hipLaunchKernelGGL(loss_final_kernel, dim3(1), dim3(256), 0, stream, c, partB, gridA, partC, n_cls);
  DY_CHECK_LAUNCH();
  return DY_OK;
}
```

### experiment-yolo_amd/ultralytics/hip/__init__.py

```python
from __future__ import annotations

import ctypes as C
import os
import sys

_FLAG = "DEBUG_CLR_GRAPH_PACKET_CAPTURE"


def _hip_already_up():
    t = sys.modules.get("torch")
    try:
        return bool(t is not None and t.cuda.is_initialized())
    except Exception:
        return False


if os.environ.get(_FLAG) is None and not _hip_already_up():
    os.environ[_FLAG] = "0"
GRAPH_SAFE = os.environ.get(_FLAG) == "0"

_HERE = os.path.dirname(os.path.abspath(__file__))
LIB_PATH = os.environ.get("DY_HIP_LIB") or os.path.normpath(os.path.join(_HERE, "..", "..", "csrc", "libdealyolo_hip.so"))

DY_EPI_STATS, DY_EPI_BIAS, DY_EPI_SILU, DY_EPI_F32OUT, DY_EPI_ACCUM, DY_EPI_STATS_ACC = 1, 2, 4, 8, 16, 32
# ... 13 lines not shown
                ("H", i32 * 4), ("W", i32 * 4), ("stride", f32 * 4),
                ("t_batch_idx", vp), ("t_cls", vp), ("t_boxes", vp), ("n_targets", i32), ("n_targets_dev", vp),
                ("img_w", f32), ("img_h", f32), ("hyp_box", f32), ("hyp_cls", f32), ("hyp_dfl", f32),
                ("use_wiou", i32), ("use_nwd", i32), ("iou_ratio", f32), ("gscale", vp), ("scalars", vp),
                ("workspace", vp), ("dbox_rows_only", i32), ("box_from_input", i32), ("box_in", vp * 4), ("box_in_ld", i32 * 4),
                ("box_w", vp * 4), ("box_b", vp * 4), ("box_in_coef", vp * 4),
                ("box_family", i32), ("box_ltype", i32), ("box_fm", i32), ("box_modifier", i32), ("inner_ratio", f32),
                ("focaler_d", f32), ("focaler_u", f32), ("shape_scale", f32), ("piou_lambda", f32)]


class DySegs(C.Structure):
    _fields_ = [("nseg", i32), ("c_end", i32 * 8), ("ld", i32 * 8), ("acc", i32 * 8), ("ptr", vp * 8)]


SIGNATURES = {
    "dy_abi_version": (i32, []),
    "dy_loss_args_bytes": (i32, []),
    "dy_conv_geometry": (i32, [i32, i32, i32, i32, ip, ip, ip, ip, ip, ip, ip, ip]),
    "dy_pack_weights": (i32, [vp, vp, vp, i32, i32, i32, i32, i32, vp]),
    "dy_pack_desc_bytes": (i32, []),
    "dy_pack_desc_fill": (i32, [vp, vp, vp, vp, i32, i32, i32, i32, i32, i32, i32, i32]),
    "dy_pack_weights_batched": (i32, [vp, i32, i32, vp]),
    "dy_conv_forward": (i32, [vp, i32, vp, vp, vp, i32, vp, i32, i32, i32, i32, i32, i32, i32, i32, i32, i32, i32, ip, vp]),
    "dy_segs_bytes": (i32, []),
    "dy_conv1x1_segs_supported": (i32, [i32, i32, C.POINTER(DySegs)]),
    "dy_conv1x1_forward_segs": (i32, [C.POINTER(DySegs), vp, vp, vp, i32, vp, i32, i32, i32, i32, i32, i32, vp]),
    "dy_conv1x1_input_grad_segs": (i32, [vp, i32, vp, C.POINTER(DySegs), i32, i32, i32, i32, i32, vp]),
    "dy_conv1x1_wgrad_bn_segs": (i32, [C.POINTER(DySegs), vp, i32, vp, i32, vp, vp, vp, vp, vp, f32, vp, vp, i32, i32, i32, i32, i32, i32, vp]),
    "dy_conv_res_supported": (i32, [i32, i32, i32, i32]),
    "dy_conv_forward_res": (i32, [vp, i32, vp, vp, vp, i32, vp, i32, i32, i32, i32, i32, i32, i32, i32, vp]),
    "dy_conv_red_supported": (i32, [i32, i32, i32]),
    "dy_conv_input_grad_red": (i32, [vp, i32, vp, vp, i32, i32, i32, i32, i32, i32, i32, vp, i32, vp, vp, i32, vp]),
    "dy_conv_kernel_name": (i32, [i32, i32, i32, i32, C.c_char_p, i32]),
    "dy_conv1x1_segs_kernel_name": (i32, [i32, i32, C.POINTER(DySegs), C.c_char_p, i32]),
    "dy_conv1x1_kernel_name_live": (i32, [i32, i32, i32, i32, i32, i32, C.POINTER(DySegs), C.POINTER(DySegs), C.c_char_p, i32]),
    "dy_conv_kernel_name_at": (i32, [i32, i32, i32, i32, i32, i32, i32, C.c_char_p, i32]),
    "dy_wgrad_kernel_name": (i32, [i32, i32, i32, i32, C.c_char_p, i32]),
    "dy_wgrad_kernel_name_at": (i32, [i32, i32, i32, i32, i32, i32, i32, C.c_char_p, i32]),
    "dy_wgrad_reduce_desc_bytes": (i32, []),
    "dy_wgrad_reduce_desc_fill": (i32, [vp, vp, i32, vp, i32, i32, i32, i32, i32, i32, i32, i32, i32]),
    "dy_wgrad_reduce_batched": (i32, [vp, i32, i32, vp]),
    "dy_match_predictions": (i32, [vp, vp, vp, vp, vp, i32, vp, vp, i32, i32, i32, i32, vp, vp, vp, vp]),
    "dy_box_iou": (i32, [vp, i32, vp, i32, vp, vp]),
    "dy_conv_num_partials": (i32, [i32, i32, i32, i32, i32, i32, i32, i32]),
    "dy_wgrad_workspace": (i32, [i32, i32, i32, i32, i32, i32, i32, ip, lp]),
    "dy_conv_wgrad": (i32, [vp, i32, vp, i32, vp, vp, i32, i32, i32, i32, i32, i32, i32, i32, vp]),
    "dy_stem_grid": (i32, [i32, i32, i32]),
    "dy_stem_forward": (i32, [vp, vp, vp, i32, vp, i32, i32, i32, f32, vp]),
    "dy_stem_forward_eval": (i32, [vp, vp, vp, vp, i32, i32, i32, i32, f32, i32, vp]),
    "dy_stem_wgrad_bn": (i32, [vp, vp, i32, vp, i32, vp, vp, vp, vp, f32, vp, i32, i32, i32, f32, vp]),
    "dy_conv_wgrad_bias": (i32, [vp, i32, vp, i32, vp, vp, vp, i32, i32, i32, i32, i32, i32, i32, i32, vp]),
    "dy_wgrad_reduce_desc_bias": (i32, [vp, vp, vp, i32]),
    "dy_conv_wgrad_bn": (i32, [vp, i32, vp, i32, vp, i32, vp, vp, vp, vp, vp, f32, vp, vp, i32, i32, i32, i32, i32, i32, i32, i32, vp]),
    "dy_conv_wgrad_ld_bn": (i32, [vp, i32, vp, i32, vp, i32, vp, vp, vp, vp, vp, f32, vp, vp, i32, i32, i32, i32, i32, i32, i32, i32, vp]),
    "dy_ldconv_sample": (i32, [vp, i32, vp, i32, vp, vp, i32, i32, i32, i32, i32, i32, i32, i32, i32, vp]),
    "dy_ldconv_sample_backward": (i32, [vp, i32, vp, i32, vp, vp, i32, vp, vp, i32, i32, i32, i32, i32, i32, i32, i32, i32, vp]),
    "dy_ldconv_sample_backward_gather": (i32, [vp, i32, vp, i32, vp, vp, i32, vp, i32, i32, vp, vp, i32, vp, i32, i32, i32, i32, i32, i32, i32, i32, i32, vp]),
    "dy_f32_to_f16_add": (i32, [vp, vp, i32, i64, i32, i32, vp]),
    "dy_pack_weights_ld": (i32, [vp, vp, i32, i32, i32, i32, i32, vp]),
    "dy_conv_wgrad_ld": (i32, [vp, i32, vp, i32, vp, vp, i32, i32, i32, i32, i32, i32, i32, i32, vp]),
    "dy_bn_finalize": (i32, [vp, i32, f32, vp, i32, f32, vp, i32, f32, vp, vp, vp, vp, vp, i32, f32, f32, f32, i32, vp]),
    "dy_bn_eval_coef": (i32, [vp, vp, vp, vp, vp, i32, f32, vp]),
    "dy_bn_act_apply": (i32, [vp, i32, vp, i32, vp, i32, vp, i64, i32, i32, vp]),
    "dy_bn_act_apply_acc": (i32, [vp, i32, vp, i32, vp, i32, vp, vp, vp, vp, vp, vp, i64, i32, i32, f32, f32, f32, vp]),
    "dy_bn_act_bwd_reduce_acc": (i32, [vp, i32, vp, i32, vp, vp, i64, i32, i32, vp, i32, i32, vp]),
    "dy_bn_act_bwd_apply_acc": (i32, [vp, i32, vp, i32, vp, i32, vp, vp, vp, vp, i64, i32, i32, f32, vp]),
    "dy_bn_act_bwd_reduce": (i32, [vp, i32, vp, i32, vp, vp, i32, i64, i32, i32, ip, vp]),
    "dy_bn_bwd_finalize": (i32, [vp, i32, vp, vp, vp, i32, f32, i32, vp]),
    "dy_bn_act_bwd_apply": (i32, [vp, i32, vp, i32, vp, i32, vp, vp, i64, i32, i32, i32, vp]),
    "dy_import_image": (i32, [vp, vp, i32, i32, i32, i32, i32, f32, vp]),
    "dy_crop_letterbox_u8": (i32, [vp, i32, i32, vp, vp, i32, i32, vp, vp]),
    "dy_refine_select": (i32, [vp, vp, vp, vp, vp, i32, C.c_float, C.c_float, vp, vp, vp]),
    "dy_nms_hard": (i32, [vp, vp, vp, i32, C.c_float, vp, vp]),
    "dy_crop_letterbox_u8_multi": (i32, [vp, vp, vp, vp, vp, vp, i32, i32, vp, vp]),
    "dy_refine_select_multi": (i32, [vp, vp, vp, vp, vp, vp, vp, i32, vp, vp, vp]),
    "dy_two_stage_merge": (i32, [vp, vp, vp, vp, vp, vp, i32, f32, vp, vp, f32, i32, vp, vp, vp, vp]),
    "dy_tile_gather_f32": (i32, [vp, vp, vp, vp, vp, vp, vp, i32, i32, vp, vp]),
    "dy_tile_merge": (i32, [vp, vp, vp, vp, vp, i32, i32, i32, f32, i32, i32, vp, vp, vp, vp, vp]),
    "dy_warp_import_u8": (i32, [vp, vp, vp, i32, i32, i32, vp]),
    "dy_warp_slot_bytes": (i32, []),
    "dy_import_image_u8": (i32, [vp, vp, i32, i32, i32, i32, vp, vp, vp, vp]),
    "dy_add": (i32, [vp, i32, vp, i32, vp, i32, vp, i32, i64, i32, vp]),
    "dy_upsample2x": (i32, [vp, i32, vp, i32, i32, i32, i32, i32, i32, i32, vp]),
    "dy_space_to_depth": (i32, [vp, i32, vp, i32, i32, i32, i32, i32, i32, i32, vp]),
    "dy_dysample_supported": (i32, [i32, i32, i32]),
    "dy_dysample": (i32, [vp, i32, vp, i32, vp, i32, i32, i32, i32, i32, i32, i32, vp]),
    "dy_dysample_backward": (i32, [vp, i32, vp, i32, vp, i32, vp, i32, i32, vp, vp, i32, vp, i32, i32, i32, i32, i32, i32, i32, vp]),
    "dy_maxpool5": (i32, [vp, i32, vp, i32, vp, i32, i32, i32, i32, vp]),
    "dy_maxpool5_backward": (i32, [vp, i32, vp, vp, i32, i32, i32, i32, i32, i32, vp]),
    "dy_bn_group_max": (i32, []),
    "dy_bn_act_apply_acc_split": (i32, [vp, i32, vp, i32, vp, i32, i32, vp, vp, vp, vp, vp, vp, i64, i32, i32, f32, f32, f32, vp]),
    "dy_bn_act_bwd_reduce_acc_split": (i32, [vp, i32, vp, i32, i32, vp, i32, vp, vp, i64, i32, i32, vp]),
    "dy_conv1x1_wgrad_bn_planes": (i32, [C.POINTER(DySegs), vp, i32, vp, vp, i32, i32, vp, i32, vp, vp, vp, vp, vp, f32, vp, vp, i32, i32, i32,
                                         i32, i32, i32, vp]),
    "dy_conv1x1_wgrad_dgrad_supported": (i32, [i32, i32, i32, i32, i32]),
    "dy_wgrad_dgrad_kernel_name": (i32, [i32, i32, i32, i32, i32, i32, C.c_char_p, i32]),
    "dy_conv1x1_wgrad_dgrad_bn": (i32, [vp, i32, vp, i32, vp, i32, vp, vp, vp, vp, f32, vp, vp, vp, vp, i32, i32, i32, i32, i32, i32, i32, i32, vp]),
    "dy_conv1x1_wgrad_dgrad_bn_segs": (i32, [C.POINTER(DySegs), vp, i32, vp, i32, vp, vp, vp, vp, f32, vp, vp, vp, C.POINTER(DySegs), i32, i32,
                                             i32, i32, i32, i32, vp]),
    "dy_conv1x1_wgrad_dgrad_bn_planes": (i32, [C.POINTER(DySegs), vp, i32, vp, vp, i32, i32, vp, i32, vp, vp, vp, vp, f32, vp, vp, vp, vp, i32, i32,
                                               C.POINTER(DySegs), i32, i32, i32, i32, i32, i32, vp]),
    "dy_conv1x1_dgrad_bn_supported": (i32, [i32, i32, i32, i32, i32]),
    "dy_dgrad_only_kernel_name": (i32, [i32, i32, i32, i32, i32, i32, C.c_char_p, i32]),
    "dy_conv1x1_dgrad_bn": (i32, [vp, vp, i32, i32, vp, i32, vp, vp, f32, vp, vp, i32, i32, C.POINTER(DySegs), i32, i32, i32, i32, i32, vp]),
    "dy_bn_act_apply_acc_group": (i32, [i32, vp, vp, vp, vp, vp, vp, vp, vp, vp, vp, vp, vp, vp, vp, vp, vp]),
    "dy_bn_act_bwd_reduce_acc_group": (i32, [i32, vp, vp, vp, vp, vp, vp, vp, vp, vp]),
# ... 76 lines not shown
```

### experiment-yolo_amd/ultralytics/hip/engine.py

```python
from __future__ import annotations

import ctypes as C
import os

import numpy as np
import torch

from . import (DY_ACT_LEAKY, DY_ACT_NONE, DY_ACT_SILU, DY_BN_COPIES, DY_EPI_ACCUM, DY_EPI_BIAS, DY_EPI_F32OUT, DY_EPI_SILU,
               DY_EPI_STATS, DY_EPI_STATS_ACC, DySegs, check, lib)

BN2D_EPS, BN2D_MOM = 1e-3, 0.03
BN3D_EPS, BN3D_MOM = 1e-5, 0.1


def _ptr(t):
    return 0 if t is None else t.data_ptr()


POISON = os.environ.get("DY_POISON", "0") == "1"

BN_ACC = os.environ.get("DY_BN_ACC", "1") != "0"
BN_WGRAD = BN_ACC and os.environ.get("DY_BN_WGRAD", "1") != "0"
STEM_DIRECT = BN_WGRAD and os.environ.get("DY_STEM_DIRECT", "1") != "0"
BN_RES = BN_ACC and os.environ.get("DY_BN_RES", "1") != "0"
# ... 755 lines not shown
                se = 9 * 16 * 16
                deferred = self.deferred_wgrad is not None
                slabs = self.transient((ns * se,), torch.float32) if deferred else self.scratch("slabs", ns * se * 4)
                self.hold(slabs)
                self.call("dy_stem_wgrad_bn", x.img.data_ptr(), y.gptr, y.ld, raw.ptr, raw.ld, spec.coef.data_ptr(), spec.acc_b.data_ptr(),
                          spec.gbn_w.data_ptr(), spec.gbn_b.data_ptr(), float(npix), slabs.data_ptr(), x.N, x.H, x.W, x.mul)
                if deferred:
                    self.deferred_wgrad.append((spec, slabs, ns))
                else:
                    keep, self.deferred_wgrad = self.deferred_wgrad, [(spec, slabs, ns)]
                    self.flush_wgrad()
                    self.deferred_wgrad = keep
            self.tape.append(bwd)
        return y

    def conv_bn_act_group(self, members, defer=None):
        defer = list(defer) if defer is not None else [False] * len(members)
        ok = (BN_GROUP and self.training and self.tape is not None and 1 < len(members) <= self.L.dy_bn_group_max()
              and all(sp.acc_f is not None and sp.acc_b is not None and sp.act == DY_ACT_SILU and sp.ld is None and not isinstance(x, ImageAct)
                      and self._live(sp, x) for sp, x in members))
        if not ok:
            return [self.conv_bn_act(sp, x, defer_apply=d) for (sp, x), d in zip(members, defer)]
        outs = []
        for (spec, x), d in zip(members, defer):
            assert x.C == spec.cin_phys, (spec.name, x.C, spec.cin_phys)
            Ho, Wo = self.out_hw(spec, x)
            raw = self.new_act(x.N, Ho, Wo, spec.cout)
            y = self.new_act(x.N, Ho, Wo, spec.cout)
            self._use(x)
            self._prod[(id(y.st), y.c0, y.C)] = (spec, raw)
            self._conv_raw(spec, x, raw.ptr, raw.ld, DY_EPI_STATS | DY_EPI_STATS_ACC, self._acc_ready(spec.acc_f))
            outs.append((spec, x, raw, y, bool(d)))
        P, I, Lg, F = C.c_void_p, C.c_int, C.c_long, C.c_float
        bn = [sp.bn for sp, *_ in outs]
        npx = [y.npix for _, _, _, y, _ in outs]
        self.call("dy_bn_act_apply_acc_group", len(outs), self._arr(P, [raw.ptr for _, _, raw, _, _ in outs]), self._arr(I, [raw.ld for _, _, raw, _, _ in outs]),
                  self._arr(P, [y.ptr for _, _, _, y, _ in outs]), self._arr(I, [y.ld for _, _, _, y, _ in outs]),
                  self._arr(P, [sp.acc_f.data_ptr() for sp, *_ in outs]), self._arr(P, [b["weight"].data_ptr() for b in bn]),
                  self._arr(P, [b["bias"].data_ptr() for b in bn]), self._arr(P, [b["running_mean"].data_ptr() for b in bn]),
                  self._arr(P, [b["running_var"].data_ptr() for b in bn]), self._arr(P, [sp.coef.data_ptr() for sp, *_ in outs]),
                  self._arr(Lg, [0 if d else n for n, (*_, d) in zip(npx, outs)]), self._arr(I, [sp.cout for sp, *_ in outs]),
                  self._arr(F, [float(n) for n in npx]), self._arr(F, [sp.bn_eps for sp, *_ in outs]), self._arr(F, [sp.bn_mom for sp, *_ in outs]))
        for spec, x, raw, y, d in outs:
            if d:
                self._unapplied[(id(y.st), y.c0, y.C)] = (raw, spec)

        def bwd():
            dense = []
            for spec, x, raw, y, _ in outs:
                assert y.grad_ready(), f"gradient of {spec.name} output incomplete"
                ykey = (id(y.st), y.c0, y.C)
                rows = self._rows_grad.get(ykey)
                if rows is not None and self._gw.get(ykey) == 1:
                    asg, A, a0 = rows
                    self.call("dy_bn_act_bwd_reduce_rows", y.gptr, y.ld, raw.ptr, raw.ld, spec.coef.data_ptr(), self._acc_ready(spec.acc_b),
                              y.N, y.H * y.W, spec.cout, spec.act, asg, A, a0)
                else:
                    dense.append((spec, raw, y))
            if len(dense) == 1:
                spec, raw, y = dense[0]
                self.call("dy_bn_act_bwd_reduce_acc", y.gptr, y.ld, raw.ptr, raw.ld, spec.coef.data_ptr(), self._acc_ready(spec.acc_b), y.npix,
                          spec.cout, spec.act, 0, 0, 0)
            elif dense:
                self.call("dy_bn_act_bwd_reduce_acc_group", len(dense), self._arr(P, [y.gptr for _, _, y in dense]), self._arr(I, [y.ld for _, _, y in dense]),
                          self._arr(P, [raw.ptr for _, raw, _ in dense]), self._arr(I, [raw.ld for _, raw, _ in dense]),
                          self._arr(P, [sp.coef.data_ptr() for sp, _, _ in dense]), self._arr(P, [self._acc_ready(sp.acc_b) for sp, _, _ in dense]),
                          self._arr(Lg, [y.npix for _, _, y in dense]), self._arr(I, [sp.cout for sp, _, _ in dense]))
            for spec, x, raw, y, _ in reversed(outs):
                self._conv_bn_act_bwd(spec, x, raw, y, None, reduced=True)
        self.tape.append(bwd)
        return [y for _, _, _, y, _ in outs]

    def _conv_bn_act_bwd(self, spec, x, raw, y, res, reduced=False):
        if isinstance(y, SegAct):
            y0, y1 = y.parts
            assert y0.grad_ready() and y1.grad_ready(), f"gradient of {spec.name} output incomplete"
            assert y1.gptr - y0.gptr == y0.npix * y0.ld * 2 and y0.ld == y1.ld == y0.C, "the planes' gradients are not one allocation"
            npix = y0.npix
            self.call("dy_bn_act_bwd_reduce_acc_split", y0.gptr, y0.ld, y1.gptr, y1.ld, y0.C, raw.ptr, raw.ld, spec.coef.data_ptr(),
                      self._acc_ready(spec.acc_b), npix, spec.cout, spec.act)
            if not spec.trainable and self._dgrad_only_ok(spec, x):
                self._dgrad_only(spec, x, raw, y0.gptr, y0.ld, npix, planes=(y1.gptr, y0.C))
                return
            if self._wgrad_dgrad_ok(spec, x):
                draw = None
            elif self.cur_sid:
                draw = self.transient((npix * spec.cout,), torch.float16)
                self.hold(draw)
            else:
                draw = self.scratch("draw", npix * spec.cout * 2)
            bn = (raw, draw, spec.coef.data_ptr(), spec.acc_b.data_ptr(), spec.gbn_w.data_ptr(), spec.gbn_b.data_ptr(), float(npix))
            self._conv_bwd(spec, x, y0.gptr, y0.ld, y0.H, y0.W, bn=bn, planes=(y1.gptr, y0.C))
            return
        assert y.grad_ready(), f"gradient of {spec.name} output incomplete"
        npix = y.npix
        acc = BN_ACC and spec.acc_b is not None
        fused_red = id(spec) in self._reduced
        if fused_red and self._gw.get((id(y.st), y.c0, y.C)) != 1:
            raise RuntimeError(f"{spec.name}: BatchNorm backward reduce was fused into a dgrad that is not the only writer of the gradient")
        rg = (0, 0, 0)
        if res is not None and res.needs_grad:
            racc = res.grad_target()
            if acc and BN_RES and res.C == spec.cout and not fused_red:
                rg = (res.gptr, res.ld, racc)
            elif racc:
                self.call("dy_add", res.gptr, res.ld, y.gptr, y.ld, 0, 0, res.gptr, res.ld, npix, res.C)
            else:
                self.call("dy_copy_slice", y.gptr, y.ld, res.gptr, res.ld, npix, res.C)
        ykey = (id(y.st), y.c0, y.C)
        rows = self._rows_grad.get(ykey)
        if rows is not None and self._gw.get(ykey) != 1:
            rows = None
        if acc and (fused_red or reduced):
            pass
        elif acc and rows is not None and rg == (0, 0, 0):
            asg, A, a0 = rows
            self.call("dy_bn_act_bwd_reduce_rows", y.gptr, y.ld, raw.ptr, raw.ld, spec.coef.data_ptr(), self._acc_ready(spec.acc_b),
                      y.N, y.H * y.W, spec.cout, spec.act, asg, A, a0)
        elif acc:
            self.call("dy_bn_act_bwd_reduce_acc", y.gptr, y.ld, raw.ptr, raw.ld, spec.coef.data_ptr(), self._acc_ready(spec.acc_b),
                      npix, spec.cout, spec.act, *rg)
        else:
            part = self.scratch("partials", 2048 * 2 * spec.cout * 4 + 4096)
            n = C.c_int(0)
            self.call("dy_bn_act_bwd_reduce", y.gptr, y.ld, raw.ptr, raw.ld, spec.coef.data_ptr(), part.data_ptr(), 2048, npix,
                      spec.cout, spec.act, C.byref(n))
            self.call("dy_bn_bwd_finalize", part.data_ptr(), n.value, spec.gbn_w.data_ptr(), spec.gbn_b.data_ptr(),
                      spec.bwdcoef.data_ptr(), spec.cout, float(npix), 0)
        frozen = not spec.trainable
        if frozen:
            if not x.needs_grad:
                return
            if acc and spec.act == DY_ACT_SILU and self._dgrad_only_ok(spec, x):
                self._dgrad_only(spec, x, raw, y.gptr, y.ld, npix)
                return
        side_small = bool(not frozen and SIDE_SMALL and npix <= SIDE_SMALL and self.deferred_wgrad is not None and not self.cur_sid and not self.side_wgrad
                          and acc and isinstance(x, Act) and x.needs_grad and spec.ld is None)
        bn_wgrad = bool(not frozen and acc and BN_WGRAD and spec.act == DY_ACT_SILU and not self.side_wgrad and not side_small and raw.ld == spec.cout)
        if bn_wgrad and self._wgrad_dgrad_ok(spec, x):
            draw = None
        elif ((self.side_wgrad or side_small) and self.deferred_wgrad is not None) or self.cur_sid:
            draw = self.transient((npix * spec.cout,), torch.float16)
            self.hold(draw)
        else:
            draw = self.scratch("draw", npix * spec.cout * 2)
        if bn_wgrad:
            bn = (raw, draw, spec.coef.data_ptr(), spec.acc_b.data_ptr(), spec.gbn_w.data_ptr(), spec.gbn_b.data_ptr(), float(npix))
            self._conv_bwd(spec, x, y.gptr, y.ld, y.H, y.W, bn=bn)
            return
        if acc:
            self.call("dy_bn_act_bwd_apply_acc", y.gptr, y.ld, raw.ptr, raw.ld, draw.data_ptr(), spec.cout, spec.coef.data_ptr(),
                      spec.acc_b.data_ptr(), spec.gbn_w.data_ptr(), spec.gbn_b.data_ptr(), npix, spec.cout, spec.act, float(npix))
        else:
            self.call("dy_bn_act_bwd_apply", y.gptr, y.ld, raw.ptr, raw.ld, draw.data_ptr(), spec.cout, spec.coef.data_ptr(),
                      spec.bwdcoef.data_ptr(), npix, spec.cout, spec.act, 0)
        self._conv_bwd(spec, x, draw.data_ptr(), spec.cout, y.H, y.W, side_hint=side_small, wgrad=not frozen)

    def _dgrad_only_ok(self, spec, x):
        if not (FROZEN_DGRAD and BN_ACC and spec.bn is not None and spec.acc_b is not None and spec.act == DY_ACT_SILU and spec.ks == 1
                and spec.stride == 1 and spec.ld is None and isinstance(x, (Act, SegAct)) and x.needs_grad
                and spec.cout == spec.cout_phys and spec.cin == spec.cin_phys):
            return False
        return bool(self.L.dy_conv1x1_dgrad_bn_supported(x.N, x.H, x.W, spec.cin, spec.cout))

    def _dgrad_only(self, spec, x, raw, dy_ptr, lddy, npix, planes=None):
        if isinstance(x, SegAct):
            accs = [q.grad_target() if q.needs_grad else 0 for q in x.parts]
            dxs, dx = C.byref(self._segs(x, grad=True, acc=accs)), (0, 0, 0)
        else:
            acc = x.grad_target()
            dxs, dx = None, (x.gptr, x.ld, int(acc))
        self.call("dy_conv1x1_dgrad_bn", dy_ptr, planes[0] if planes else 0, lddy, planes[1] if planes else 0, raw.ptr, raw.ld,
                  spec.coef.data_ptr(), spec.acc_b.data_ptr(), float(npix), spec.wpack_t.data_ptr(), *dx, dxs, x.N, x.H, x.W, spec.cin, spec.cout)

    def _wgrad_dgrad_ok(self, spec, x):
        if not (WGRAD_DGRAD and spec.ks == 1 and spec.stride == 1 and spec.ld is None and isinstance(x, (Act, SegAct)) and x.needs_grad
                and not self.cur_sid and not self.side_wgrad and spec.cout == spec.cout_phys and spec.cin == spec.cin_phys):
            return False
        return bool(self.L.dy_conv1x1_wgrad_dgrad_supported(x.N, x.H, x.W, spec.cin, spec.cout))

    def _conv_bwd(self, spec, x, dy_ptr, lddy, Ho, Wo, accumulate_w=0, defer=True, bn=None, bias_acc=None, planes=None, side_hint=False,
                  wgrad=True):
        if not wgrad:
            assert bn is None and bias_acc is None and planes is None
            return self._input_grad(spec, x, dy_ptr, lddy, Ho, Wo)
        ns, se = C.c_int(), C.c_long()
        self.L.dy_wgrad_workspace(x.N, x.H, x.W, spec.cin, spec.cout, spec.ks, spec.stride, C.byref(ns), C.byref(se))
        deferred = defer and not accumulate_w and self.deferred_wgrad is not None
        if self.wgrad_log is not None and not deferred:
            self.wgrad_log.append(spec)
        if deferred:
            slabs = self.transient((ns.value * se.value,), torch.float32)
            self.hold(slabs)
            self.deferred_wgrad.append((spec, slabs, ns.value) if bias_acc is None else (spec, slabs, ns.value, bias_acc))
            dw = 0
        else:
            slabs = self.scratch("slabs", ns.value * se.value * 4)
            dw = spec.gweight.data_ptr()
        side = deferred and (self.side_wgrad or side_hint)
        if side:
            self._side_used = True
            self.fork()
        if bn is not None and bn[1] is None:
            raw, _, coef, accb, gw, gb, cnt = bn
            assert not side and self._wgrad_dgrad_ok(spec, x)
            seg = isinstance(x, SegAct)
            if seg:
                accs = [q.grad_target() if q.needs_grad else 0 for q in x.parts]
                dxs, dx = C.byref(self._segs(x, grad=True, acc=accs)), (0, 0, 0)
            else:
                acc = x.grad_target()
                dxs, dx = None, (x.gptr, x.ld, int(acc))
            tail = (x.N, x.H, x.W, spec.cin, spec.cout, accumulate_w)
            wt = spec.wpack_t.data_ptr()
            if planes is not None:
                self.call("dy_conv1x1_wgrad_dgrad_bn_planes", C.byref(self._segs(x)) if seg else None, 0 if seg else x.ptr, 0 if seg else x.ld,
                          dy_ptr, planes[0], lddy, planes[1], raw.ptr, raw.ld, coef, accb, gw, gb, cnt, slabs.data_ptr(), dw, wt, *dx, dxs, *tail)
            elif seg:
                self.call("dy_conv1x1_wgrad_dgrad_bn_segs", C.byref(self._segs(x)), dy_ptr, lddy, raw.ptr, raw.ld, coef, accb, gw, gb, cnt,
                          slabs.data_ptr(), dw, wt, dxs, *tail)
            else:
                self.call("dy_conv1x1_wgrad_dgrad_bn", x.ptr, x.ld, dy_ptr, lddy, raw.ptr, raw.ld, coef, accb, gw, gb, cnt, slabs.data_ptr(), dw,
                          wt, *dx, *tail)
            return
        if planes is not None:
            raw, draw, coef, accb, gw, gb, cnt = bn
            seg = isinstance(x, SegAct)
            self.call("dy_conv1x1_wgrad_bn_planes", C.byref(self._segs(x)) if seg else None, 0 if seg else x.ptr, 0 if seg else x.ld, dy_ptr,
                      planes[0], lddy, planes[1], raw.ptr, raw.ld, draw.data_ptr() if x.needs_grad else 0, coef, accb, gw, gb, cnt,
                      slabs.data_ptr(), dw, x.N, x.H, x.W, spec.cin, spec.cout, accumulate_w)
            dy_ptr, lddy = draw.data_ptr(), spec.cout
        elif bn is not None and isinstance(x, SegAct):
            raw, draw, coef, accb, gw, gb, cnt = bn
            self.call("dy_conv1x1_wgrad_bn_segs", C.byref(self._segs(x)), dy_ptr, lddy, raw.ptr, raw.ld, draw.data_ptr() if x.needs_grad else 0,
                      coef, accb, gw, gb, cnt, slabs.data_ptr(), dw, x.N, x.H, x.W, spec.cin, spec.cout, accumulate_w)
            dy_ptr, lddy = draw.data_ptr(), spec.cout
        elif bn is not None:
            raw, draw, coef, accb, gw, gb, cnt = bn
            head = (x.ptr, x.ld, dy_ptr, lddy, raw.ptr, raw.ld, draw.data_ptr() if x.needs_grad else 0, coef, accb, gw, gb, cnt,
                    slabs.data_ptr(), dw, x.N, x.H, x.W)
            if spec.ld is not None:
                n, cphys, cin = spec.ld
                self.call("dy_conv_wgrad_ld_bn", *head, spec.cout, cin, n, cphys, accumulate_w)
            else:
                self.call("dy_conv_wgrad_bn", *head, spec.cin, spec.cout, spec.ks, spec.stride, accumulate_w)
            dy_ptr, lddy = draw.data_ptr(), spec.cout
        elif bias_acc is not None:
            assert deferred
            self.call("dy_conv_wgrad_bias", x.ptr, x.ld, dy_ptr, lddy, self._acc_ready(bias_acc), slabs.data_ptr(), dw, x.N, x.H, x.W,
                      spec.cin, spec.cout, spec.ks, spec.stride, accumulate_w)
        elif spec.ld is not None:
            n, cphys, cin = spec.ld
            self.call("dy_conv_wgrad_ld", x.ptr, x.ld, dy_ptr, lddy, slabs.data_ptr(), dw, x.N, x.H, x.W,
                      spec.cout, cin, n, cphys, accumulate_w, side=side)
        else:
            self.call("dy_conv_wgrad", x.ptr, x.ld, dy_ptr, lddy, slabs.data_ptr(), dw, x.N, x.H, x.W,
                      spec.cin, spec.cout, spec.ks, spec.stride, accumulate_w, side=side)
        if isinstance(x, SegAct):
            assert bn is not None, f"{spec.name}: a segmented input needs the BatchNorm-in-the-weight-gradient path"
        self._input_grad(spec, x, dy_ptr, lddy, Ho, Wo)

    wgrad_log = None

    def _input_grad(self, spec, x, dy_ptr, lddy, Ho, Wo):
        if isinstance(x, SegAct):
            if x.needs_grad:
                accs = [q.grad_target() if q.needs_grad else 0 for q in x.parts]
                self.call("dy_conv1x1_input_grad_segs", dy_ptr, lddy, spec.wpack_t.data_ptr(), C.byref(self._segs(x, grad=True, acc=accs)),
                          x.N, Ho, Wo, spec.cout_phys, spec.cin)
            return
        if x.needs_grad:
            acc = x.grad_target()
            prod = self._sole_consumer_of_conv(x) if (BN_DGRED and not acc and spec.stride == 1 and spec.ld is None) else None
            if prod is not None:
                ps, praw = prod
                if not (ps.act == DY_ACT_SILU and ps.acc_b is not None and ps.cout == x.C == spec.cin and x.C <= BN_DGRED_MAXC and x.npix <= BN_DGRED_MAXPIX
                        and (praw.N, praw.H, praw.W) == (x.N, x.H, x.W)
                        and self.L.dy_conv_red_supported(spec.cout_phys, spec.cin, spec.ks)):
                    prod = None
            if prod is not None:
                self.call("dy_conv_input_grad_red", dy_ptr, lddy, spec.wpack_t.data_ptr(), x.gptr, x.ld, x.N, Ho, Wo, spec.cout_phys, spec.cin,
                          spec.ks, praw.ptr, praw.ld, ps.coef.data_ptr(), self._acc_ready(ps.acc_b), ps.cout)
                self._reduced.add(id(ps))
            else:
                self.call("dy_conv_forward", dy_ptr, lddy, spec.wpack_t.data_ptr(), 0, x.gptr, x.ld, 0, x.N, Ho, Wo,
                          spec.cout_phys, spec.cin, spec.ks, 1, spec.stride, x.H, x.W, DY_EPI_ACCUM if acc else 0, None)

    deferred_wgrad = None
    tape_mark = None

    def flush_wgrad(self):
        items, self.deferred_wgrad = self.deferred_wgrad, None
        if self.side_wgrad or self._side_used:
            self.join()
            self._side_used = False
        if not items:
# ... 46 lines not shown
        live = self._live(spec, x)
        if live:
            self._use(x)
        self._conv_raw(spec, x, y_ptr, ldy, DY_EPI_BIAS | (DY_EPI_F32OUT if f32out else 0), 0, spec.bias)
        if self.tape is not None and live:
            if (rows_level is not None and self.rows_used is not None and spec.ks == 1 and spec.ld is None and spec.acc_bias is not None
                    and self.L.dy_conv1x1_rows_supported(spec.cin, spec.cout)):
                self.rows_used.add(rows_level)
            else:
                rows_level = None
            self.tape.append(lambda: self._conv_bias_bwd(spec, x, dy_ptr_fn, rows_level=rows_level))

    def rows_capable(self, spec):
        return (self.rows_used is not None and self.tape is not None and spec.ks == 1 and spec.ld is None and spec.acc_bias is not None
                and spec.bias is not None and bool(self.L.dy_conv1x1_rows_supported(spec.cin, spec.cout)))

    def cls_capable(self, spec, ncp):
        return (HEAD_CLS and self.pending_decode is not None and self.tape is not None and spec.ks == 1 and spec.ld is None and ncp == 8
                and spec.acc_bias is not None and spec.bias is not None and bool(self.L.dy_cls_head_supported(spec.cin, spec.cout)))

    def conv_bias_cls(self, spec: ConvSpec, x: Act, y_ptr, dy_ptr_fn):
        self._use(x)
        src = self.unapplied(x)
        xp, xld, xcoef = (x.ptr, x.ld, 0) if src is None else (src[0].ptr, src[0].ld, src[1].coef.data_ptr())
        self.call("dy_cls_head_forward", xp, xld, xcoef, spec.weight.data_ptr(), spec.bias.data_ptr(), y_ptr, x.npix, spec.cin, spec.cout)

        def bwd():
            dyp, ld = dy_ptr_fn()
            assert ld == 8 and self.deferred_wgrad is not None and not self.side_wgrad
            ns = self.L.dy_cls_head_slabs()
            slabs = self.transient((ns * 16 * spec.cin,), torch.float32)
            self.hold(slabs)
            self.deferred_wgrad.append((spec, slabs, ns, spec.acc_bias))
            acc = x.grad_target() if x.needs_grad else 0
            self.call("dy_cls_head_backward", xp, xld, xcoef, dyp, spec.weight.data_ptr(), x.gptr if x.needs_grad else 0, x.ld, acc,
                      slabs.data_ptr(), self._acc_ready(spec.acc_bias), x.npix, spec.cin, spec.cout)
        self.tape.append(bwd)

    @staticmethod
    def _arr(ctype, vals):
        return (ctype * len(vals))(*vals)

    def _src(self, x):
        src = self.unapplied(x)
        return (x.ptr, x.ld, 0) if src is None else (src[0].ptr, src[0].ld, src[1].coef.data_ptr())

    def head_box_levels(self, items, dy_ptr_fns):
        for spec, x, l in items:
            self._use(x)
            self.rows_used.add(l)
            self.pending_decode.append((spec, x, l))
        self.tape.append(lambda: self._rows_bwd_levels(items, dy_ptr_fns))

    def _rows_bwd_levels(self, items, fns):
        if not (self.loss_rows is not None and self.deferred_wgrad is not None and not self.side_wgrad):
            for (spec, x, l), fn in zip(items, fns):
                self._conv_bias_bwd(spec, x, fn, rows_level=l)
            return
        asg, A, a0 = self.loss_rows
        cols = {k: [] for k in ("x", "ldx", "xc", "dy", "lddy", "a0", "w", "dx", "lddx", "acc", "slabs", "bacc", "h", "w_")}
        for (spec, x, l), fn in zip(items, fns):
            dyp, ld = fn()
            Ho, Wo = self.out_hw(spec, x)
            ns = self.L.dy_conv1x1_rows_slabs(x.N, Ho, Wo)
            slabs = self.transient((ns * spec.cout * spec.cin,), torch.float32)
            self.hold(slabs)
            self.deferred_wgrad.append((spec, slabs, ns, spec.acc_bias))
            acc = x.grad_target() if x.needs_grad else 0
            if x.needs_grad and not acc and self._sole_consumer_of_conv(x) is not None:
                self._rows_grad[(id(x.st), x.c0, x.C)] = (asg, A, a0[l])
            xp, xld, xc = self._src(x)
            for k, v in zip(cols, (xp, xld, xc, dyp, ld, a0[l], spec.weight.data_ptr(), x.gptr if x.needs_grad else 0, x.ld, acc,
                                   slabs.data_ptr(), self._acc_ready(spec.acc_bias), Ho, Wo)):
                cols[k].append(v)
        P, I = C.c_void_p, C.c_int
        spec0, x0 = items[0][0], items[0][1]
        self.call("dy_conv1x1_rows_backward_levels", len(items), self._arr(P, cols["x"]), self._arr(I, cols["ldx"]), self._arr(P, cols["xc"]),
                  self._arr(P, cols["dy"]), self._arr(I, cols["lddy"]), asg, A, self._arr(I, cols["a0"]), self._arr(P, cols["w"]),
                  self._arr(P, cols["dx"]), self._arr(I, cols["lddx"]), self._arr(I, cols["acc"]), self._arr(P, cols["slabs"]),
                  self._arr(P, cols["bacc"]), x0.N, self._arr(I, cols["h"]), self._arr(I, cols["w_"]), spec0.cin, spec0.cout)

    def head_cls_levels(self, items):
        P, I, Lg = C.c_void_p, C.c_int, C.c_long
        srcs = [self._src(x) for _, x, _, _ in items]
        for _, x, _, _ in items:
            self._use(x)
        spec0 = items[0][0]
        self.call("dy_cls_head_forward_levels", len(items), self._arr(P, [s_[0] for s_ in srcs]), self._arr(I, [s_[1] for s_ in srcs]),
                  self._arr(P, [s_[2] for s_ in srcs]), self._arr(P, [sp.weight.data_ptr() for sp, _, _, _ in items]),
                  self._arr(P, [sp.bias.data_ptr() for sp, _, _, _ in items]), self._arr(P, [yp for _, _, yp, _ in items]),
                  self._arr(Lg, [x.npix for _, x, _, _ in items]), spec0.cin, spec0.cout)

        def bwd():
            assert self.deferred_wgrad is not None and not self.side_wgrad
            dys, dxs, accs, slabs_l, baccs = [], [], [], [], []
            ns = self.L.dy_cls_head_slabs()
            for spec, x, _, fn in items:
                dyp, ld = fn()
                assert ld == 8
                slabs = self.transient((ns * 16 * spec.cin,), torch.float32)
                self.hold(slabs)
                self.deferred_wgrad.append((spec, slabs, ns, spec.acc_bias))
                accs.append(x.grad_target() if x.needs_grad else 0)
                dys.append(dyp); dxs.append(x.gptr if x.needs_grad else 0); slabs_l.append(slabs.data_ptr())
                baccs.append(self._acc_ready(spec.acc_bias))
            self.call("dy_cls_head_backward_levels", len(items), self._arr(P, [s_[0] for s_ in srcs]), self._arr(I, [s_[1] for s_ in srcs]),
                      self._arr(P, [s_[2] for s_ in srcs]), self._arr(P, dys), self._arr(P, [sp.weight.data_ptr() for sp, _, _, _ in items]),
                      self._arr(P, dxs), self._arr(I, [x.ld for _, x, _, _ in items]), self._arr(I, accs), self._arr(P, slabs_l),
                      self._arr(P, baccs), self._arr(Lg, [x.npix for _, x, _, _ in items]), spec0.cin, spec0.cout)
        self.tape.append(bwd)

    def unapplied(self, x):
        return self._unapplied.get((id(x.st), x.c0, x.C))

    def conv_bias_decode(self, spec: ConvSpec, x: Act, dy_ptr_fn, rows_level):
        self._use(x)
        self.rows_used.add(rows_level)
        self.pending_decode.append((spec, x, rows_level))
        self.tape.append(lambda: self._conv_bias_bwd(spec, x, dy_ptr_fn, rows_level=rows_level))

    infer_head = False
    pending_decode = None
    rows_used = None
    loss_rows = None

    def _conv_bias_bwd(self, spec, x, dy_ptr_fn, accumulate=0, defer=True, rows_level=None):
        dyp, ld = dy_ptr_fn()
        Ho, Wo = self.out_hw(spec, x)
        if (rows_level is not None and self.loss_rows is not None and defer and not accumulate and self.deferred_wgrad is not None
                and not self.side_wgrad):
            asg, A, a0 = self.loss_rows
            ns = self.L.dy_conv1x1_rows_slabs(x.N, Ho, Wo)
            slabs = self.transient((ns * spec.cout * spec.cin,), torch.float32)
            self.hold(slabs)
            self.deferred_wgrad.append((spec, slabs, ns, spec.acc_bias))
            acc = x.grad_target() if x.needs_grad else 0
            if x.needs_grad and not acc and self._sole_consumer_of_conv(x) is not None:
                self._rows_grad[(id(x.st), x.c0, x.C)] = (asg, A, a0[rows_level])
            src = self.unapplied(x)
            xp, xld, xcoef = (x.ptr, x.ld, 0) if src is None else (src[0].ptr, src[0].ld, src[1].coef.data_ptr())
            self.call("dy_conv1x1_rows_backward", xp, xld, xcoef, dyp, ld, asg, A, a0[rows_level], spec.weight.data_ptr(),
                      x.gptr if x.needs_grad else 0, x.ld, acc, slabs.data_ptr(), self._acc_ready(spec.acc_bias), x.N, Ho, Wo,
                      spec.cin, spec.cout)
            return
        assert self.unapplied(x) is None, f"{spec.name}: the dense backward needs the activated input that was never written"
        if (BIAS_WGRAD and defer and not accumulate and self.deferred_wgrad is not None and spec.acc_bias is not None and spec.ld is None
                and not self.side_wgrad):
            self._conv_bwd(spec, x, dyp, ld, Ho, Wo, bias_acc=spec.acc_bias)
            return
        npix = x.N * Ho * Wo
        cp = spec.cout_phys
        part = self.scratch("partials", 2048 * 2 * cp * 4 + 4096)
        n = C.c_int(0)
        ident = self.ident_coef(cp)
        self.call("dy_bn_act_bwd_reduce", dyp, ld, dyp, ld, ident.data_ptr(), part.data_ptr(), 2048, npix, cp, DY_ACT_NONE,
                  C.byref(n))
        tmp = self.scratch("bwdcoef_tmp", 2 * cp * 4)
        self.call("dy_bn_bwd_finalize", part.data_ptr(), n.value, 0, spec.gbias.data_ptr(), tmp.data_ptr(), cp, 1.0, accumulate)
        self._conv_bwd(spec, x, dyp, ld, Ho, Wo, accumulate, defer=defer)

    def upsample2x(self, x: Act, out: Act | None = None):
        x = self.dense(x)
        if UPSEG and PLANAR and out is None and x.st.buf.dtype == torch.float16 and (self.tape is None or UPSEG_TRAIN):
            up = UpAct(x)
            if self.tape is not None and x.needs_grad:
                self._use(x)

                def bwd():
                    if up._g is None or not up._g.st.gwritten:
                        assert up._full is not None, "an up-sampled tensor without a consumer"
                        return
                    assert up.grad_ready(), "gradient of an up-sampled concat member incomplete"
                    acc = x.grad_target()
                    self.call("dy_upsample2x", up.gptr, up.gld, x.gptr, x.ld, x.N, x.H, x.W, x.C, 1, acc)
                self.tape.append(bwd)
            return up
        return self._upsample_now(x, out)

    def _upsample_now(self, x: Act, out: Act | None = None, optional=False):
        y = out if out is not None else self.new_act(x.N, 2 * x.H, 2 * x.W, x.C)
        self._use(x)
        self.call("dy_upsample2x", x.ptr, x.ld, y.ptr, y.ld, x.N, x.H, x.W, x.C, 0, 0)

        def bwd():
            if optional and not y.st.gwritten:
                return
            acc = x.grad_target()
            self.call("dy_upsample2x", y.gptr, y.ld, x.gptr, x.ld, x.N, x.H, x.W, x.C, 1, acc)
        self._record(self._live(None, x), y, bwd)
        return y

# ... 314 lines not shown
```

### experiment-yolo_amd/ultralytics/hip/train.py

```python
from __future__ import annotations

import ctypes as C
import math
import os
import sys

import numpy as np
import torch
import torch.distributed as dist

from . import check, lib
from .dist import all_reduce_flat
from .engine import Recorder


class StepPlan:
    def __init__(self, model, batch_size, imgsz, nmax=16, optimizer="SGD", hyp=None, world_size=1, use_graph=False,
                 init_scale=65536.0, side_wgrad=None, dynamic_scale=True, share=None, arena=None, input_act=False):
        self.model = model
        self.arena = arena
        self.side_wgrad = bool(int(os.environ.get("DY_SIDE_WGRAD", "0"))) if side_wgrad is None else bool(side_wgrad)
        dev = next(model.parameters()).device
        self.rt = model._runtime(dev)
        self.eng = self.rt.eng
# ... 566 lines not shown
        for _ in range(reps):
            torch.cuda._sleep(60_000_000)
            evs[0].record()
            for i, (fn, args, name, _side) in enumerate(ops):
                rc = fn(*args, s)
                if rc != 0:
                    check(rc, name)
                evs[i + 1].record()
            torch.cuda.synchronize()
            for i in range(len(ops)):
                tot[i] += evs[i].elapsed_time(evs[i + 1])
        cal = [torch.cuda.Event(enable_timing=True) for _ in range(33)]
        torch.cuda._sleep(20_000_000)
        for e in cal:
            e.record()
        torch.cuda.synchronize()
        gaps = sorted(cal[i].elapsed_time(cal[i + 1]) for i in range(32))
        self.event_gap_ms = gaps[len(gaps) // 2]
        return [(ops[i][2], ops[i][1], max(tot[i] / reps - self.event_gap_ms, 0.0)) for i in range(len(ops))]

    @staticmethod
    def conv_algorithmic_bytes(args):
        (_x, _ldx, _w, _b, _y, _ldy, _p, n, h, w, cin, cout, ks, stride, dil, oh, ow, epi, _np) = args
        H, W = (2 * h, 2 * w) if dil == 2 else (h, w)
        pad = ks // 2
        Ho, Wo = ((H + 2 * pad - ks) // stride + 1, (W + 2 * pad - ks) // stride + 1) if not oh else (oh, ow)
        ob = 4 if epi & 8 else 2
        out = n * Ho * Wo * cout * ob
        return n * h * w * cin * 2 + out * (2 if epi & 16 else 1)

    @staticmethod
    def wgrad_algorithmic_bytes(args):
        (_x, _ldx, _dy, _lddy, _sl, _dw, n, h, w, cin, cout, ks, stride, _acc) = args[:14]
        pad = ks // 2
        Ho, Wo = (h + 2 * pad - ks) // stride + 1, (w + 2 * pad - ks) // stride + 1
        return n * h * w * ((cin + 7) // 8 * 8) * 2 + n * Ho * Wo * ((cout + 7) // 8 * 8) * 2

    def kernel_of(self, name, args):
        key, alg = self._kernel_alg(name, args)
        own = alg
        e = 2
        if name == "dy_bn_act_apply":
            own = int(args[7]) * int(args[8]) * e * (3 if args[2] else 2)
        elif name == "dy_bn_act_apply_acc":
            own = int(args[12]) * int(args[13]) * e * (3 if args[2] else 2)
        elif name == "dy_bn_act_bwd_reduce":
            own = int(args[7]) * int(args[8]) * e * 2
        elif name == "dy_bn_act_bwd_reduce_acc":
            own = int(args[6]) * int(args[7]) * e * (2 + ((2 if args[11] else 1) if args[9] else 0))
        elif name == "dy_bn_act_bwd_apply":
            own = int(args[8]) * int(args[9]) * e * 3
        elif name == "dy_bn_act_bwd_apply_acc":
            own = int(args[10]) * int(args[11]) * e * 3
        elif name in ("dy_conv_wgrad_bn", "dy_conv_wgrad_ld_bn"):
            n, h, w = args[14:17]
            if name == "dy_conv_wgrad_bn":
                cin, cout, ks, stride = args[17:21]
            else:
                cout, ks, stride = args[17], 1, 1
            pad = ks // 2
            own = alg + 2 * n * ((h + 2 * pad - ks) // stride + 1) * ((w + 2 * pad - ks) // stride + 1) * ((cout + 7) // 8 * 8) * e
        elif name == "dy_stem_wgrad_bn":
            n, h, w = args[11:14]
            own = alg + n * ((h - 1) // 2 + 1) * ((w - 1) // 2 + 1) * 16 * e
        elif name in ("dy_conv1x1_wgrad_bn_segs", "dy_conv1x1_wgrad_bn_planes") and alg:
            n, h, w, _cin, cout = args[13:18] if name.endswith("segs") else args[17:22]
            own = alg + 2 * n * h * w * ((cout + 7) // 8 * 8) * e
        elif name in self._FUSED_BWD and alg:
            n, h, w, cin, cout, old = self._fused_bwd_shape(name, args)
            own = n * h * w * (2 * cin + 2 * cout + old) * e
        elif name == "dy_bn_act_apply_acc_split":
            own = int(args[13]) * int(args[14]) * e * 2
        elif name == "dy_bn_act_bwd_reduce_acc_split":
            own = int(args[9]) * int(args[10]) * e * 2
        return key, alg, own

    _FUSED_BWD = {"dy_conv1x1_wgrad_dgrad_bn": 17, "dy_conv1x1_wgrad_dgrad_bn_segs": 14, "dy_conv1x1_wgrad_dgrad_bn_planes": 21}

    def _fused_bwd_shape(self, name, args):
        i = self._FUSED_BWD[name]
        n, h, w, cin, cout = args[i:i + 5]
        dxs = args[13] if name.endswith("segs") else (args[20] if name.endswith("planes") else None)
        if dxs is not None:
            t = dxs._obj
            old = sum((t.c_end[k] - (t.c_end[k - 1] if k else 0)) for k in range(t.nseg) if t.acc[k])
        else:
            old = cin if args[16 if name.endswith("bn") else 19] else 0
        return n, h, w, cin, cout, old

    def _kernel_alg(self, name, args):
        import ctypes as C
        L, buf = self.eng.L, C.create_string_buffer(128)
        if name in self._FUSED_BWD:
            n, h, w, cin, cout, old = self._fused_bwd_shape(name, args)
            seg = name.endswith("segs") or (name.endswith("planes") and args[0] is not None)
            if L.dy_wgrad_dgrad_kernel_name(n, h, w, cin, cout, int(seg), buf, 128) == 0:
                return buf.value.decode(), n * h * w * (2 * (cin + cout) + (0 if seg else old)) * 2
        if name == "dy_conv1x1_dgrad_bn":
            n, h, w, cin, cout = args[14:19]
            if L.dy_dgrad_only_kernel_name(n, h, w, cin, cout, int(args[13] is not None), buf, 128) == 0:
                return buf.value.decode(), n * h * w * (cin + cout) * 2
        if name == "dy_conv_forward":
            n, h, w, cin, cout, ks, stride, dil = args[7:15]
            if dil == 2 and ks == 3:
                return f"conv_mfma_dg2_kernel (input gradient of the {cout}->{cin} stride-2 3x3)", self.conv_algorithmic_bytes(args)
            pad = ks // 2
            if ks == 1 and L.dy_conv1x1_kernel_name_live(cin, cout, n, h, w, int(args[17]), None, None, buf, 128) == 0:
                return buf.value.decode(), self.conv_algorithmic_bytes(args)
            if L.dy_conv_kernel_name_at(cin, cout, ks, stride, (w + 2 * pad - ks) // stride + 1, dil, int(args[17]), buf, 128) == 0:
                return buf.value.decode(), self.conv_algorithmic_bytes(args)
        if name == "dy_conv1x1_forward_segs":
            n, h, w, cin, cout = args[6:11]
            if L.dy_conv1x1_kernel_name_live(cin, cout, n, h, w, int(args[11]), args[0], None, buf, 128) == 0:
                return buf.value.decode(), n * h * w * (cin + (cout + 7) // 8 * 8) * 2
        if name == "dy_conv1x1_input_grad_segs":
            n, h, w, cin, cout = args[4:9]
            if L.dy_conv1x1_kernel_name_live(cin, cout, n, h, w, 0, None, args[3], buf, 128) == 0:
                return buf.value.decode(), n * h * w * (cin + cout) * 2
        if name in ("dy_conv1x1_wgrad_bn_segs", "dy_conv1x1_wgrad_bn_planes"):
            n, h, w, cin, cout = args[13:18] if name.endswith("segs") else args[17:22]
            if L.dy_wgrad_kernel_name_at(n, h, w, cin, cout, 1, 1, buf, 128) == 0:
                seg = args[0] is not None
                return buf.value.decode().replace(", 0>", ", 3>" if seg else ", 1>"), n * h * w * (cin + (cout + 7) // 8 * 8) * 2
        if name == "dy_conv_wgrad":
            n, h, w, cin, cout, ks, stride = args[6:13]
            if L.dy_wgrad_kernel_name_at(n, h, w, cin, cout, ks, stride, buf, 128) == 0:
                return buf.value.decode(), self.wgrad_algorithmic_bytes(args)
        if name == "dy_conv_input_grad_red":
            n, h, w, cin, cout, ks = args[5:11]
            if L.dy_conv_kernel_name(cin, cout, ks, 1, buf, 128) == 0:
                return buf.value.decode().replace("false, 0>", "true, 0>"), n * h * w * (cin + cout) * 2
        if name == "dy_stem_forward":
            n, h, w = args[5:8]
            return "stem_fwd_kernel", n * h * w * 3 * 2 + n * ((h - 1) // 2 + 1) * ((w - 1) // 2 + 1) * 16 * 2
        if name == "dy_stem_wgrad_bn":
            n, h, w = args[11:14]
            return "stem_wgrad_bn_kernel", n * h * w * 3 * 2 + n * ((h - 1) // 2 + 1) * ((w - 1) // 2 + 1) * 16 * 2
        if name in ("dy_conv_wgrad_bn", "dy_conv_wgrad_ld_bn"):
            n, h, w = args[14:17]
            if name == "dy_conv_wgrad_bn":
                cin, cout, ks, stride = args[17:21]
            else:
                cout, _ld_cin, ld_taps, ld_cphys = args[17:21]
                cin, ks, stride = ld_taps * ld_cphys, 1, 1
            if L.dy_wgrad_kernel_name_at(n, h, w, cin, cout, ks, stride, buf, 128) == 0:
                pad = ks // 2
                Ho, Wo = (h + 2 * pad - ks) // stride + 1, (w + 2 * pad - ks) // stride + 1
                return (buf.value.decode().replace(", 0>", ", 1>"),
                        n * h * w * ((cin + 7) // 8 * 8) * 2 + n * Ho * Wo * ((cout + 7) // 8 * 8) * 2)
        if name == "dy_conv_wgrad_ld":
            n, h, w, cout, ld_cin, ld_taps, ld_cphys = args[6:13]
            if L.dy_wgrad_kernel_name_at(n, h, w, ld_taps * ld_cphys, cout, 1, 1, buf, 128) == 0:
                return buf.value.decode(), n * h * w * (ld_taps * ld_cphys + (cout + 7) // 8 * 8) * 2
        tmpl = {"dy_bn_act_apply": ("bn_act_apply_kernel<{}, false, false>", 9), "dy_bn_act_apply_acc": ("bn_act_apply_kernel<{}, true, " + ("false" if os.environ.get("DY_SILU_FAST") == "0" else "true") + ">", 14),
                "dy_bn_act_bwd_reduce": ("bn_act_bwd_reduce_kernel<{}, false>", 9),
                "dy_bn_act_bwd_apply": ("bn_act_bwd_apply_kernel<{}, false>", 10),
                "dy_bn_act_bwd_apply_acc": ("bn_act_bwd_apply_kernel<{}, true>", 12)}
        if name == "dy_bn_act_bwd_reduce_acc":
            return f"bn_act_bwd_reduce_kernel<{int(args[8])}, {'true' if args[9] else 'false'}>", 0
        if name == "dy_bn_act_bwd_reduce_acc_split":
            return f"bn_act_bwd_reduce_kernel<{int(args[11])}, false>", 0
        if name == "dy_bn_act_apply_acc_split":
            return f"bn_act_apply_kernel<{int(args[15])}, true, true>", 0
        if name in tmpl:
            k, i = tmpl[name]
            return k.format(int(args[i])), 0
        return name.replace("dy_", "", 1) + " (C-ABI call)", 0

    def probe_dominant_kernel(self, batch, reps=10):
        if self.rec_fb is None:
            self.forward_backward(batch)
        prof = self.profile_ops(reps)
        self.last_profile = prof
        groups = {}
        for name, args, ms in prof:
            key, by, own = self.kernel_of(name, args)
            groups.setdefault(key, []).append((ms, by, own))

        def summary(key):
            items = groups[key]
            ms = sum(t[0] for t in items) / len(items)
            by = sum(t[2] for t in items) / len(items)
            return {"kernel": key, "us": ms * 1e3, "bytes": by, "gbs": by / (ms * 1e-3) / 1e9 if ms > 0 else 0.0,
                    "algorithmic_bytes": sum(t[1] for t in items) / len(items),
                    "launches_per_step": len(items), "ms_per_step": sum(t[0] for t in items)}

        if not groups:
            return None
        rank = sorted(groups, key=lambda k: -sum(t[0] for t in groups[k]))
        top = summary(rank[0])
        convs = [k for k in rank if k.startswith("conv_")]
        top["top_conv"] = summary(convs[0]) if convs else None
        algs = [k for k in rank if sum(t[1] for t in groups[k]) > 0]
        if algs:
            ta = summary(algs[0])
            ta["alg_gbs"] = ta["algorithmic_bytes"] / (ta["us"] * 1e-6) / 1e9 if ta["us"] > 0 else 0.0
            top["top_alg"] = ta
        else:
            top["top_alg"] = None
        top["ranking"] = [{"kernel": k, "ms_per_step": round(sum(t[0] for t in groups[k]), 4), "launches": len(groups[k]),
                           "algorithmic_MB_per_step": round(sum(t[1] for t in groups[k]) / 1e6, 1),
# ... 13 lines not shown
```

### include/dealyolo_hip.h

```cpp
#ifndef DEALYOLO_HIP_H
#define DEALYOLO_HIP_H

#include <stddef.h>
#include <stdint.h>

#ifdef __cplusplus
extern "C" {
#endif

#ifndef __HIP__
typedef struct ihipStream_t* hipStream_t;
#endif

#define DY_OK 0
#define DY_ERR_ARG (-1)
#define DY_ERR_LAUNCH (-2)
#define DY_ERR_ALIGN (-3)
#define DY_ERR_CAPACITY (-4)

#define DY_MAX_SEGS 8
typedef struct DySegs {
  int nseg;
  int c_end[DY_MAX_SEGS];
  int ld[DY_MAX_SEGS];
  int acc[DY_MAX_SEGS];
  const void* ptr[DY_MAX_SEGS];
} DySegs;
int dy_segs_bytes(void);

#define DY_EPI_STATS 1
#define DY_EPI_BIAS 2
#define DY_EPI_SILU 4
#define DY_EPI_F32OUT 8
#define DY_EPI_ACCUM 16
#define DY_EPI_STATS_ACC 32
#define DY_BN_COPIES 16

#define DY_ACT_NONE 0
#define DY_ACT_SILU 1
#define DY_ACT_LEAKY 2

int dy_abi_version(void);

int dy_conv_geometry(int cin, int cout, int ks, int stride, int* cin_p, int* cout_p, int* cc, int* nch, int* mt,
                     int* ngroups, int* ksteps, int* packed_elems);
int dy_pack_weights(const float* w, const float* scale, void* out, int cout, int cin, int ks, int stride,
                    int transposed, hipStream_t stream);
int dy_pack_desc_bytes(void);
int dy_pack_desc_fill(void* desc, const float* w, const float* scale, void* out, int cout, int cin, int ks, int stride,
                      int transposed, int ld_taps, int ld_cphys, int first_block);
int dy_pack_weights_batched(const void* descs_device, int n, int total_blocks, hipStream_t stream);
int dy_conv_forward(const void* x, int ldx, const void* w_packed, const float* bias, void* y, int ldy, float* partials,
                    int n, int h, int w, int cin, int cout, int ks, int stride, int dil, int out_h, int out_w, int epi,
                    int* num_partials, hipStream_t stream);
int dy_conv_num_partials(int n, int h, int w, int cin, int cout, int ks, int stride, int dil);
int dy_conv_res_supported(int cin, int cout, int ks, int stride);
int dy_conv_forward_res(const void* x, int ldx, const void* w_packed, const float* bias, const void* res, int ldres, void* y, int ldy,
                        int n, int h, int w, int cin, int cout, int ks, int stride, hipStream_t stream);
int dy_conv_red_supported(int cin, int cout, int ks);
int dy_conv_input_grad_red(const void* dy, int lddy, const void* w_packed_t, void* dx, int lddx, int n, int h, int w, int cin, int cout,
                           int ks, const void* raw, int ldraw, const float* coef, double* acc, int C, hipStream_t stream);
int dy_conv_kernel_name(int cin, int cout, int ks, int stride, char* out, int cap);
int dy_conv_kernel_name_at(int cin, int cout, int ks, int stride, int out_w, int dil, int epi, char* out, int cap);

int dy_wgrad_workspace(int n, int h, int w, int cin, int cout, int ks, int stride, int* nslabs, long* slab_elems);
int dy_wgrad_kernel_name(int cin, int cout, int ks, int stride, char* out, int cap);
int dy_wgrad_kernel_name_at(int n, int h, int w, int cin, int cout, int ks, int stride, char* out, int cap);
int dy_conv_wgrad(const void* x, int ldx, const void* dy, int lddy, float* slabs, float* dw, int n, int h, int w,
                  int cin, int cout, int ks, int stride, int accumulate, hipStream_t stream);
int dy_conv_wgrad_bn(const void* x, int ldx, const void* dy, int lddy, const void* raw, int ldraw, void* draw, const float* coef,
                     const double* acc, float* dgamma, float* dbeta, float count, float* slabs, float* dw, int n, int h, int w,
                     int cin, int cout, int ks, int stride, int accumulate, hipStream_t stream);
int dy_conv_wgrad_ld_bn(const void* x, int ldx, const void* dy, int lddy, const void* raw, int ldraw, void* draw,
                        const float* coef, const double* acc, float* dgamma, float* dbeta, float count, float* slabs, float* dw,
                        int n, int h, int w, int cout, int ld_cin, int ld_taps, int ld_cphys, int accumulate, hipStream_t stream);
int dy_conv1x1_segs_supported(int cin, int cout, const DySegs* xs);
int dy_conv1x1_segs_kernel_name(int cin, int cout, const DySegs* xs, char* out, int cap);
int dy_conv1x1_kernel_name_live(int cin, int cout, int n, int h, int w, int epi, const DySegs* xs, const DySegs* ys, char* out, int cap);
int dy_conv1x1_forward_segs(const DySegs* xs, const void* w_packed, const float* bias, void* y, int ldy, float* partials, int n, int h,
                            int w, int cin, int cout, int epi, hipStream_t stream);
int dy_conv1x1_input_grad_segs(const void* dy, int lddy, const void* w_packed_t, const DySegs* dxs, int n, int h, int w, int cin, int cout,
                               hipStream_t stream);
int dy_conv1x1_wgrad_bn_segs(const DySegs* xs, const void* dy, int lddy, const void* raw, int ldraw, void* draw, const float* coef,
                             const double* acc, float* dgamma, float* dbeta, float count, float* slabs, float* dw, int n, int h, int w,
                             int cin, int cout, int accumulate, hipStream_t stream);
int dy_bn_act_apply_acc_split(const void* x, int ldx, void* y, int ldy, void* y2, int ldy2, int csplit, const double* acc,
                              const float* gamma, const float* beta, float* running_mean, float* running_var, float* coef, long npix,
                              int C, int act, float count, float eps, float momentum, hipStream_t stream);
int dy_bn_act_bwd_reduce_acc_split(const void* dy, int lddy, const void* dy2, int lddy2, int csplit, const void* x, int ldx,
                                   const float* coef, double* acc, long npix, int C, int act, hipStream_t stream);
int dy_conv1x1_wgrad_bn_planes(const DySegs* xs, const void* x, int ldx, const void* dy, const void* dy2, int lddy, int csplit,
                               const void* raw, int ldraw, void* draw, const float* coef, const double* acc, float* dgamma,
                               float* dbeta, float count, float* slabs, float* dw, int n, int h, int w, int cin, int cout,
                               int accumulate, hipStream_t stream);
int dy_conv1x1_wgrad_dgrad_supported(int n, int h, int w, int cin, int cout);
int dy_wgrad_dgrad_kernel_name(int n, int h, int w, int cin, int cout, int segs, char* out, int cap);
int dy_conv1x1_wgrad_dgrad_bn(const void* x, int ldx, const void* dy, int lddy, const void* raw, int ldraw, const float* coef,
                              const double* acc, float* dgamma, float* dbeta, float count, float* slabs, float* dw,
                              const void* w_packed_t, void* dx, int lddx, int dx_accumulate, int n, int h, int w, int cin, int cout,
                              int accumulate, hipStream_t stream);
int dy_conv1x1_wgrad_dgrad_bn_segs(const DySegs* xs, const void* dy, int lddy, const void* raw, int ldraw, const float* coef,
                                   const double* acc, float* dgamma, float* dbeta, float count, float* slabs, float* dw,
                                   const void* w_packed_t, const DySegs* dxs, int n, int h, int w, int cin, int cout, int accumulate,
                                   hipStream_t stream);
int dy_conv1x1_wgrad_dgrad_bn_planes(const DySegs* xs, const void* x, int ldx, const void* dy, const void* dy2, int lddy, int csplit,
                                     const void* raw, int ldraw, const float* coef, const double* acc, float* dgamma, float* dbeta,
                                     float count, float* slabs, float* dw, const void* w_packed_t, void* dx, int lddx,
                                     int dx_accumulate, const DySegs* dxs, int n, int h, int w, int cin, int cout, int accumulate,
                                     hipStream_t stream);
int dy_conv1x1_dgrad_bn_supported(int n, int h, int w, int cin, int cout);
int dy_dgrad_only_kernel_name(int n, int h, int w, int cin, int cout, int segs, char* out, int cap);
int dy_conv1x1_dgrad_bn(const void* dy, const void* dy2, int lddy, int csplit, const void* raw, int ldraw, const float* coef,
                        const double* acc, float count, const void* w_packed_t, void* dx, int lddx, int dx_accumulate,
                        const DySegs* dxs, int n, int h, int w, int cin, int cout, hipStream_t stream);
int dy_stem_grid(int n, int h, int w);
int dy_stem_forward(const float* img_nchw, const float* weight, void* raw, int ldraw, double* acc, int n, int h, int w, float mul,
                    hipStream_t stream);
int dy_stem_forward_eval(const float* img_nchw, const float* weight, const float* bias, void* y, int ldy, int n, int h, int w, float mul,
                         int silu, hipStream_t stream);
int dy_stem_wgrad_bn(const float* img_nchw, const void* dy, int lddy, const void* raw, int ldraw, const float* coef,
                     const double* acc, float* dgamma, float* dbeta, float count, float* slabs, int n, int h, int w, float mul,
                     hipStream_t stream);
int dy_conv_wgrad_bias(const void* x, int ldx, const void* dy, int lddy, double* bias_acc, float* slabs, float* dw, int n, int h, int w,
                       int cin, int cout, int ks, int stride, int accumulate, hipStream_t stream);
int dy_wgrad_reduce_desc_bias(void* desc, const double* bias_acc, float* dbias, int c);
// ... 254 lines not shown
```

Before: 6127 images/s.

## Skip background rows in head backward, pipeline cls-head bwd loads, vectorize target packing

Adds a sparse head-row input-gradient kernel that writes dX only at foreground (assigned) pixels. A matching 3x3 BatchNorm wgrad variant reads dY only where the assignment flag is set, and zero-fills tiles that have no foreground. Separately, the classification-head backward gets a depth-4 software prefetch queue, and target packing counts slots with 16-byte vectorized LDS reads. Together these aim to cut gradient-traffic and latency costs. They add flag loads and a guard that errors if any consumer would read the sparse gradient densely.

Result: no change. 6172 images/s (median of 6 runs) (+0.7%).

```diff
diff --git a/experiment-yolo_amd/csrc/conv_wgrad.hip b/experiment-yolo_amd/csrc/conv_wgrad.hip
--- a/experiment-yolo_amd/csrc/conv_wgrad.hip
+++ b/experiment-yolo_amd/csrc/conv_wgrad.hip
@@ -32,6 +32,8 @@
   int lddx, dx_acc;
   int dg_mt, dg_rows;
   DySegs dxs;
+  const int* dy_flag;
+  int fA, fa0;
 };
 
 static __device__ __forceinline__ half8 tr_frag(const char* base0, const char* base1) {
@@ -59,6 +61,8 @@
   constexpr bool BN1 = ((BNF & 3) == 1 || (BNF & 3) == 3);
   constexpr bool XSEG = ((BNF & 3) == 3);
   static_assert(!DG || (KS == 1 && BN1), "the fused input gradient exists for the 1x1 BatchNorm forms");
+  constexpr bool ROWS = (BNF & 16) != 0;
+  static_assert(!ROWS || (BNF == 17 && KS == 3 && STRIDE == 1), "rows of dY: the 3x3 stride-1 BatchNorm form only");
   constexpr int TAPS = KS * KS;
   constexpr int NCOL = NCI * TAPS;
   constexpr int CPW = (NCOL + 3) / 4;
@@ -106,6 +110,8 @@
   unsigned roff[BN1 ? NPY : 1];
   int ncur = 0, nnext = 0;
   (void)ncur; (void)nnext;
+  int fnext[ROWS ? NPY : 1];
+  (void)fnext;
   unsigned vnext = 0, vcur = 0, ornext = 0, orcur = 0;
   (void)pfr; (void)roff; (void)vnext; (void)vcur; (void)ornext; (void)orcur;
   constexpr unsigned NEVER = 0x80000000u;
@@ -236,6 +242,24 @@
     const auto v = __builtin_amdgcn_raw_buffer_load_b128(r, (int)off, 0, 0);
     return *reinterpret_cast<const uint4*>(&v);
   };
+  auto load_flags = [&](int tile) {
+#pragma unroll
+    for (int i = 0; i < NPY; ++i) fnext[ROWS ? i : 0] = -1;
+    if (tile < a.ntiles) {
+      const int bx = tile % a.tiles_x;
+      const int t2 = tile / a.tiles_x;
+      const int n = t2 / a.tiles_y;
+      const int oy0 = (t2 % a.tiles_y) * TH, ox0 = bx * TW;
+      const int* const fl = a.dy_flag + (size_t)n * a.fA + a.fa0;
+#pragma unroll
+      for (int i = 0; i < NPY; ++i) {
+        const int id = tid + i * 256, pixel = id / CPGY;
+        const int ty = pixel / TW, tx = pixel - ty * TW;
+        if (id < NGY && oy0 + ty < a.Ho && ox0 + tx < a.Wo) fnext[ROWS ? i : 0] = fl[(oy0 + ty) * a.Wo + ox0 + tx];
+      }
+    }
+  };
+  (void)load_flags;
   auto prefetch = [&](int tile) {
     if (FLAT) {
       const auto rx = __builtin_amdgcn_make_buffer_rsrc(const_cast<f16*>(a.x), 0, (int)((unsigned)a.npix * (unsigned)a.ldx * 2u), 0x00020000);
@@ -303,7 +327,19 @@
           pfx[i] = ld16(rx, (unsigned)(ix0 + hx) < (unsigned)a.W ? xoff[i] + ox : NEVER);
         }
       }
-      if (ox0 + TW <= a.Wo) {
+      if (ROWS) {
+        bool any = false;
+#pragma unroll
+        for (int i = 0; i < NPY; ++i) any = any || fnext[ROWS ? i : 0] >= 0;
+        if (__builtin_amdgcn_ballot_w64(any) == 0) {
+#pragma unroll
+          for (int i = 0; i < NPY; ++i) pfy[i] = make_uint4(0, 0, 0, 0);
+        } else {
+#pragma unroll
+          for (int i = 0; i < NPY; ++i) pfy[i] = ld16(ry, fnext[ROWS ? i : 0] >= 0 ? yoff[i] + oy : NEVER);
+        }
+        load_flags(tile + (int)gridDim.x);
+      } else if (ox0 + TW <= a.Wo) {
 #pragma unroll
         for (int i = 0; i < NPY; ++i) pfy[i] = ld16(ry, yoff[i] + oy);
       } else {
@@ -336,6 +372,7 @@
 
 
   int tile = (!FLAT && !(gridDim.x & 7)) ? (int)(blockIdx.x & 7) * (int)(gridDim.x >> 3) + (int)(blockIdx.x >> 3) : (int)blockIdx.x;
+  if (ROWS) load_flags(tile);
   if (tile < a.ntiles) prefetch(tile);
   for (; tile < a.ntiles; tile += gridDim.x) {
     __syncthreads();
@@ -635,6 +672,9 @@
     } else return DY_ERR_ARG;
   } else if (a.raw && a.xs.nseg > 0) {
     if constexpr (KS == 1) hipLaunchKernelGGL((conv_wgrad_kernel<KS, STRIDE, NCI, MTC, 3>), dim3(gx, gy), dim3(256), 0, s, a);
+    else return DY_ERR_ARG;
+  } else if (a.raw && a.dy_flag) {
+    if constexpr (KS == 3 && STRIDE == 1 && NCI != 3 && MTC != 3) hipLaunchKernelGGL((conv_wgrad_kernel<KS, STRIDE, NCI, MTC, 17>), dim3(gx, gy), dim3(256), 0, s, a);
     else return DY_ERR_ARG;
   } else if (a.raw) hipLaunchKernelGGL((conv_wgrad_kernel<KS, STRIDE, NCI, MTC, 1>), dim3(gx, gy), dim3(256), 0, s, a);
   else if (a.acc && MTC != 3) hipLaunchKernelGGL((conv_wgrad_kernel<KS, STRIDE, NCI, MTC, 2>), dim3(gx, gy), dim3(256), 0, s, a);
@@ -717,6 +757,8 @@
   unsigned dy_plane = 0;
   const void* wt = nullptr; void* dx = nullptr; int lddx = 0, dx_acc = 0; const DySegs* dxs = nullptr;
   bool dgrad_only = false;
+  const int* dy_flag = nullptr;
+  int fA = 0, fa0 = 0;
 };
 static int conv_wgrad_impl(const void* x, int ldx, const void* dy, int lddy, float* slabs, float* dw, int n, int h, int w,
                            int cin, int cout, int ks, int stride, int accumulate, int ld_taps, int ld_cphys, int ld_cin,
@@ -755,6 +797,16 @@
                                 hipStream_t stream) {
   if (!raw || !coef || !acc || (ldraw & 7) || ((uintptr_t)raw & 15) || ((uintptr_t)draw & 15) || (cout & 15)) return DY_ERR_ARG;
   const WgBnHost bn{raw, draw, coef, acc, dgamma, dbeta, ldraw, count};
+  return conv_wgrad_impl(x, ldx, dy, lddy, slabs, dw, n, h, w, cin, cout, ks, stride, accumulate, 0, 0, 0, stream, &bn);
+}
+extern "C" int dy_conv_wgrad_bn_rows(const void* x, int ldx, const void* dy, int lddy, const void* raw, int ldraw, void* draw,
+                                     const float* coef, const double* acc, float* dgamma, float* dbeta, float count, float* slabs,
+                                     float* dw, int n, int h, int w, int cin, int cout, int ks, int stride, int accumulate,
+                                     const int* assigned, int A, int a0, hipStream_t stream) {
+  if (!raw || !coef || !acc || (ldraw & 7) || ((uintptr_t)raw & 15) || ((uintptr_t)draw & 15) || (cout & 15)) return DY_ERR_ARG;
+  if (ks != 3 || stride != 1 || !assigned || n < 1 || h < 1 || w < 1 || a0 < 0 || (long)a0 + (long)h * w > A) return DY_ERR_ARG;
+  WgBnHost bn{raw, draw, coef, acc, dgamma, dbeta, ldraw, count};
+  bn.dy_flag = assigned; bn.fA = A; bn.fa0 = a0;
   return conv_wgrad_impl(x, ldx, dy, lddy, slabs, dw, n, h, w, cin, cout, ks, stride, accumulate, 0, 0, 0, stream, &bn);
 }
 extern "C" int dy_conv_wgrad_bias(const void* x, int ldx, const void* dy, int lddy, double* bias_acc, float* slabs, float* dw, int n,
@@ -952,6 +1004,7 @@
     a.cout = bn->raw ? cout : (cout + 7) / 8 * 8;
     if (bn->xs) a.xs = *bn->xs;
     a.dy_csplit = bn->dy_csplit; a.dy_plane = bn->dy_plane;
+    a.dy_flag = bn->dy_flag; a.fA = bn->fA; a.fa0 = bn->fa0;
     if (bn->wt) {
       const WgDgPlan pl = wgrad_dgrad_plan(n, h, w, cin, cout);
       if (!pl.ok || pl.nci != nci || pl.mtc != mtc || ks != 1 || ld_taps) return DY_ERR_ARG;
diff --git a/experiment-yolo_amd/csrc/head_rows.hip b/experiment-yolo_amd/csrc/head_rows.hip
--- a/experiment-yolo_amd/csrc/head_rows.hip
+++ b/experiment-yolo_amd/csrc/head_rows.hip
@@ -101,7 +101,7 @@
 
 __global__ __launch_bounds__(256) void rows_dgrad_kernel(Levels<RowsArgs> L) {
   const RowsArgs& a = L.lv[blockIdx.z];
-  if (!a.dx || (int)blockIdx.x >= a.dgx || (int)blockIdx.y >= a.B) return;
+  if (!a.dx || a.dx_acc == 2 || (int)blockIdx.x >= a.dgx || (int)blockIdx.y >= a.B) return;
   __shared__ float s_w[64 * 65];
   for (int i = threadIdx.x; i < 64 * 64; i += 256) s_w[(i >> 6) * 65 + (i & 63)] = (float)(f16)a.w[i];
   __syncthreads();
@@ -137,6 +137,78 @@
       for (int k = 0; k < 8; ++k) o[k] = (f16)s[k];
     }
     *reinterpret_cast<half8*>(dst) = o;
+  }
+}
+
+__global__ __launch_bounds__(256) void rows_dgrad_sparse_kernel(Levels<RowsArgs> L) {
+  const RowsArgs& a = L.lv[blockIdx.y];
+  if (!a.dx || a.dx_acc != 2 || (int)blockIdx.x >= a.nblk) return;
+  __shared__ float s_w[64 * 65];
+  __shared__ int s_list[256];
+  __shared__ int s_cnt[4];
+  const int tid = threadIdx.x, wave = tid >> 6, lane = tid & 63;
+  for (int i = tid; i < 64 * 64; i += 256) s_w[(i >> 6) * 65 + (i & 63)] = (float)(f16)a.w[i];
+  const int ci0 = (tid & 7) * 8;
+  const long npix = (long)a.B * a.hw;
+  const long chunk = (npix + a.nblk - 1) / a.nblk;
+  const long lo = (long)blockIdx.x * chunk, hi = lo + chunk < npix ? lo + chunk : npix;
+  constexpr int FB = 8;
+  int fl[FB];
+  for (long p0 = lo, trip = 0; p0 < hi; p0 += 256, ++trip) {
+    if ((trip & (FB - 1)) == 0) {
+#pragma unroll
+      for (int k = 0; k < FB; ++k) {
+        const long pk = p0 + (long)k * 256 + tid;
+        fl[k] = -1;
+        if (pk < hi) {
+          const int b = (int)(pk / a.hw), r = (int)(pk - (long)b * a.hw);
+          fl[k] = a.flag[(size_t)b * a.A + a.a0 + r];
+        }
+      }
+    }
+    int mine = -1;
+#pragma unroll
+    for (int k = 0; k < FB; ++k)
+      if ((trip & (FB - 1)) == k) mine = fl[k];
+    const bool fg = mine >= 0;
+    const unsigned long long m = __ballot(fg);
+    if (lane == 0) s_cnt[wave] = __popcll(m);
+    __syncthreads();
+    int base = 0, total = 0;
+#pragma unroll
+    for (int w = 0; w < 4; ++w) {
+      if (w < wave) base += s_cnt[w];
+      total += s_cnt[w];
+    }
+    if (fg) s_list[base + __popcll(m & ((1ull << lane) - 1ull))] = tid;
+    __syncthreads();
+    for (int i0 = 0; i0 < total; i0 += 32) {
+      const int i = i0 + (tid >> 3);
+      if (i < total) {
+        const long p = p0 + s_list[i];
+        float s[8];
+#pragma unroll
+        for (int k = 0; k < 8; ++k) s[k] = 0.f;
+        const f16* const g = a.dy + p * a.lddy;
+        half8 gv[8];
+#pragma unroll
+        for (int c = 0; c < 8; ++c) gv[c] = *reinterpret_cast<const half8*>(g + c * 8);
+#pragma unroll
+        for (int c = 0; c < 8; ++c) {
+#pragma unroll
+          for (int j = 0; j < 8; ++j) {
+            const float gg = (float)gv[c][j];
+#pragma unroll
+            for (int k = 0; k < 8; ++k) s[k] += gg * s_w[(c * 8 + j) * 65 + ci0 + k];
+          }
+        }
+        half8 o;
+#pragma unroll
+        for (int k = 0; k < 8; ++k) o[k] = (f16)s[k];
+        *reinterpret_cast<half8*>(a.dx + p * a.lddx + ci0) = o;
+      }
+    }
+    __syncthreads();
   }
 }
 
@@ -305,7 +377,7 @@
                      const float* weight, void* dx, int lddx, int dx_accumulate, float* slabs, double* bias_acc, int n, int h, int w, int cin,
                      int cout) {
   if (!dy_conv1x1_rows_supported(cin, cout) || !x || !dy || !assigned || !weight || !slabs || !bias_acc || n < 1 || h < 1 || w < 1 ||
-      a0 < 0 || a0 + h * w > A)
+      a0 < 0 || a0 + h * w > A || dx_accumulate < 0 || dx_accumulate > 2)
     return DY_ERR_ARG;
   if ((ldx & 7) || (lddy & 7) || (dx && (lddx & 7)) || ((uintptr_t)x & 15) || ((uintptr_t)dy & 15) || ((uintptr_t)dx & 15) ||
       ((uintptr_t)slabs & 15))
@@ -317,14 +389,16 @@
   return DY_OK;
 }
 static int rows_launch(const Levels<RowsArgs>& L, hipStream_t stream) {
-  int gw = 1, gd = 0, nb = 1;
+  int gw = 1, gd = 0, gs = 0, nb = 1;
   for (int l = 0; l < L.nl; ++l) {
     gw = L.lv[l].nblk > gw ? L.lv[l].nblk : gw;
-    if (L.lv[l].dx) gd = L.lv[l].dgx > gd ? L.lv[l].dgx : gd;
+    if (L.lv[l].dx && L.lv[l].dx_acc != 2) gd = L.lv[l].dgx > gd ? L.lv[l].dgx : gd;
+    if (L.lv[l].dx && L.lv[l].dx_acc == 2) gs = L.lv[l].nblk > gs ? L.lv[l].nblk : gs;
     nb = L.lv[l].B > nb ? L.lv[l].B : nb;
   }
   hipLaunchKernelGGL(rows_wgrad_kernel, dim3(gw, L.nl), dim3(256), 0, stream, L);
   if (gd) hipLaunchKernelGGL(rows_dgrad_kernel, dim3(gd, nb, L.nl), dim3(256), 0, stream, L);
+  if (gs) hipLaunchKernelGGL(rows_dgrad_sparse_kernel, dim3(gs, L.nl), dim3(256), 0, stream, L);
   DY_CHECK_LAUNCH();
   return DY_OK;
 }
@@ -401,8 +475,8 @@
     }
   }
 }
-template <int CIN>
-__global__ __launch_bounds__(256) void cls_head_bwd_kernel(Levels<ClsArgs> L) {
+template <int CIN, int DEPTH>
+__global__ __launch_bounds__(256, DEPTH > 1 ? 2 : 1) void cls_head_bwd_kernel(Levels<ClsArgs> L) {
   const ClsArgs& a = L.lv[blockIdx.y];
   if ((int)blockIdx.x >= a.nblk) return;
   constexpr int PARTS = CIN / 8, PPB = 256 / PARTS;
@@ -426,9 +500,8 @@
   }
   const long chunk = ((a.npix + a.nblk - 1) / a.nblk + PPB - 1) / PPB * PPB;
   const long lo = (long)blockIdx.x * chunk, hi = lo + chunk < a.npix ? lo + chunk : a.npix;
-  for (long pix = lo + tid / PARTS; pix < hi; pix += PPB) {
-    half8 xv = *reinterpret_cast<const half8*>(a.x + pix * a.ldx + k0);
-    const half8 dv = *reinterpret_cast<const half8*>(a.dy + pix * 8);
+  const bool addold = a.dx && a.dx_acc;
+  auto pixel = [&](long pix, half8 xv, const half8 dv, const half8 old) {
     if (a.xcoef) xv = bn_silu_apply8(xv, sc, sh);
     float d[8], g[8];
 #pragma unroll
@@ -448,7 +521,6 @@
       f16* dst = a.dx + pix * a.lddx + k0;
       half8 o;
       if (a.dx_acc) {
-        const half8 old = *reinterpret_cast<const half8*>(dst);
 #pragma unroll
         for (int j = 0; j < 8; ++j) o[j] = (f16)((float)old[j] + g[j]);
       } else {
@@ -457,6 +529,35 @@
       }
       *reinterpret_cast<half8*>(dst) = o;
     }
+  };
+  if constexpr (DEPTH == 1) {
+    for (long pix = lo + tid / PARTS; pix < hi; pix += PPB) {
+      const half8 xv = *reinterpret_cast<const half8*>(a.x + pix * a.ldx + k0);
+      const half8 dv = *reinterpret_cast<const half8*>(a.dy + pix * 8);
+      half8 old = (half8){0, 0, 0, 0, 0, 0, 0, 0};
+      if (addold) old = *reinterpret_cast<const half8*>(a.dx + pix * a.lddx + k0);
+      pixel(pix, xv, dv, old);
+    }
+  } else {
+  half8 xq[DEPTH], dq[DEPTH], oq[DEPTH];
+  auto request = [&](int k, long pix) {
+    xq[k] = dq[k] = oq[k] = (half8){0, 0, 0, 0, 0, 0, 0, 0};
+    if (pix < hi) {
+      xq[k] = *reinterpret_cast<const half8*>(a.x + pix * a.ldx + k0);
+      dq[k] = *reinterpret_cast<const half8*>(a.dy + pix * 8);
+      if (addold) oq[k] = *reinterpret_cast<const half8*>(a.dx + pix * a.lddx + k0);
+    }
+  };
+  const long first = lo + tid / PARTS;
+#pragma unroll
+  for (int k = 0; k < DEPTH; ++k) request(k, first + (long)k * PPB);
+  for (long pix = first; pix < hi; pix += PPB) {
+    const half8 xv = xq[0], dv = dq[0], old = oq[0];
+#pragma unroll
+    for (int k = 0; k + 1 < DEPTH; ++k) { xq[k] = xq[k + 1]; dq[k] = dq[k + 1]; oq[k] = oq[k + 1]; }
+    request(DEPTH - 1, pix + (long)DEPTH * PPB);
+    pixel(pix, xv, dv, old);
+  }
   }
 #pragma unroll
   for (int c = 0; c < 8; ++c) {
@@ -497,6 +598,11 @@
     const float b = (s_bs[0][tid] + s_bs[1][tid]) + (s_bs[2][tid] + s_bs[3][tid]);
     if (b != 0.f) unsafeAtomicAdd(a.bias_acc + (size_t)(blockIdx.x % DY_BN_COPIES) * 8 + tid, (double)b);
   }
+}
+constexpr int CLS_BWD_DEPTH = 4;
+static bool cls_head_v1() {
+  const char* e = getenv("DY_CLS_HEAD_V1");
+  return e && e[0] == '1' && !e[1];
 }
 extern "C" int dy_cls_head_supported(int cin, int nc) { return (cin == 32 || cin == 64) && nc >= 1 && nc <= 8; }
 extern "C" int dy_cls_head_slabs(void) { return 512; }
@@ -522,10 +628,16 @@
   int gx = 1;
   for (int l = 0; l < L.nl; ++l) gx = L.lv[l].nblk > gx ? L.lv[l].nblk : gx;
   const dim3 grid(gx, L.nl);
+  const bool v1 = cls_head_v1();
   if (!backward && cin == 32) hipLaunchKernelGGL(cls_head_fwd_kernel<32>, grid, dim3(256), 0, stream, L);
   else if (!backward) hipLaunchKernelGGL(cls_head_fwd_kernel<64>, grid, dim3(256), 0, stream, L);
-  else if (cin == 32) hipLaunchKernelGGL(cls_head_bwd_kernel<32>, grid, dim3(256), 0, stream, L);
-  else hipLaunchKernelGGL(cls_head_bwd_kernel<64>, grid, dim3(256), 0, stream, L);
+  else if (cin == 32) {
+    if (v1) hipLaunchKernelGGL((cls_head_bwd_kernel<32, 1>), grid, dim3(256), 0, stream, L);
+    else hipLaunchKernelGGL((cls_head_bwd_kernel<32, CLS_BWD_DEPTH>), grid, dim3(256), 0, stream, L);
+  } else {
+    if (v1) hipLaunchKernelGGL((cls_head_bwd_kernel<64, 1>), grid, dim3(256), 0, stream, L);
+    else hipLaunchKernelGGL((cls_head_bwd_kernel<64, CLS_BWD_DEPTH>), grid, dim3(256), 0, stream, L);
+  }
   DY_CHECK_LAUNCH();
   return DY_OK;
 }
diff --git a/experiment-yolo_amd/csrc/loss.hip b/experiment-yolo_amd/csrc/loss.hip
--- a/experiment-yolo_amd/csrc/loss.hip
+++ b/experiment-yolo_amd/csrc/loss.hip
@@ -373,6 +373,7 @@
   }
 }
 
+template <bool V1>
 __global__ void pack_targets_kernel(LossCtx c, const float* bidx, const float* cls, const float* boxes, int n,
                                     const int* n_dev, float img_w, float img_h) {
   if (n_dev) n = *n_dev;
@@ -384,7 +385,7 @@
     for (int k = 0; k < 4; ++k) c.gt_box[i * 4 + k] = 0.f;
   }
   if (threadIdx.x == 0) c.scal[9] = 0.f;
-  __shared__ short sb[8192];
+  __shared__ __attribute__((aligned(16))) short sb[8192];
   const int ncache = n < 8192 ? n : 8192;
   for (int i = threadIdx.x; i < ncache; i += blockDim.x) sb[i] = (short)(int)bidx[i];
   __syncthreads();
@@ -392,7 +393,20 @@
     const int b = (int)bidx[i];
     if (b < 0 || b >= c.B) continue;
     int slot = 0;
-    for (int j = 0; j < i; ++j) slot += ((j < ncache ? (int)sb[j] : (int)bidx[j]) == b);
+    if (V1) {
+      for (int j = 0; j < i; ++j) slot += ((j < ncache ? (int)sb[j] : (int)bidx[j]) == b);
+    } else {
+      const int ic = i < ncache ? i : ncache;
+      int j = 0;
+      for (; j + 8 <= ic; j += 8) {
+        const uint4 v = *reinterpret_cast<const uint4*>(sb + j);
+        const unsigned wd[4] = {v.x, v.y, v.z, v.w};
+#pragma unroll
+        for (int k = 0; k < 4; ++k) slot += ((int)(short)(wd[k] & 0xffffu) == b) + ((int)(short)(wd[k] >> 16) == b);
+      }
+      for (; j < ic; ++j) slot += ((int)sb[j] == b);
+      for (j = ncache; j < i; ++j) slot += ((int)bidx[j] == b);
+    }
     if (slot >= c.nmax) {
       c.scal[9] = 1.f;
       c.scal[10] = 1.f;
@@ -1013,8 +1027,13 @@
     c.use_wiou = fam == DY_BOX_FAMILY_WISE;
   }
 
-  hipLaunchKernelGGL(pack_targets_kernel, dim3(1), dim3(1024), 0, stream, c, d->t_batch_idx, d->t_cls, d->t_boxes,
-                     d->n_targets, d->n_targets_dev, d->img_w, d->img_h);
+  const char* const pt_v1 = getenv("DY_PACK_TARGETS_V1");
+  if (pt_v1 && pt_v1[0] == '1' && !pt_v1[1])
+    hipLaunchKernelGGL(pack_targets_kernel<true>, dim3(1), dim3(1024), 0, stream, c, d->t_batch_idx, d->t_cls, d->t_boxes,
+                       d->n_targets, d->n_targets_dev, d->img_w, d->img_h);
+  else
+    hipLaunchKernelGGL(pack_targets_kernel<false>, dim3(1), dim3(1024), 0, stream, c, d->t_batch_idx, d->t_cls, d->t_boxes,
+                       d->n_targets, d->n_targets_dev, d->img_w, d->img_h);
   if (hipMemsetAsync(c.cnt, 0, BA * 4, stream) != hipSuccess) return DY_ERR_LAUNCH;
   const int gridA = (int)((BA * 64 + 255) / 256 < 2048 ? (BA * 64 + 255) / 256 : 2048);
   if (!d->box_from_input) {
diff --git a/experiment-yolo_amd/ultralytics/hip/__init__.py b/experiment-yolo_amd/ultralytics/hip/__init__.py
--- a/experiment-yolo_amd/ultralytics/hip/__init__.py
+++ b/experiment-yolo_amd/ultralytics/hip/__init__.py
@@ -89,6 +89,7 @@
     "dy_conv_wgrad_bias": (i32, [vp, i32, vp, i32, vp, vp, vp, i32, i32, i32, i32, i32, i32, i32, i32, vp]),
     "dy_wgrad_reduce_desc_bias": (i32, [vp, vp, vp, i32]),
     "dy_conv_wgrad_bn": (i32, [vp, i32, vp, i32, vp, i32, vp, vp, vp, vp, vp, f32, vp, vp, i32, i32, i32, i32, i32, i32, i32, i32, vp]),
+    "dy_conv_wgrad_bn_rows": (i32, [vp, i32, vp, i32, vp, i32, vp, vp, vp, vp, vp, f32, vp, vp, i32, i32, i32, i32, i32, i32, i32, i32, vp, i32, i32, vp]),
     "dy_conv_wgrad_ld_bn": (i32, [vp, i32, vp, i32, vp, i32, vp, vp, vp, vp, vp, f32, vp, vp, i32, i32, i32, i32, i32, i32, i32, i32, vp]),
     "dy_ldconv_sample": (i32, [vp, i32, vp, i32, vp, vp, i32, i32, i32, i32, i32, i32, i32, i32, i32, vp]),
     "dy_ldconv_sample_backward": (i32, [vp, i32, vp, i32, vp, vp, i32, vp, vp, i32, i32, i32, i32, i32, i32, i32, i32, i32, vp]),
diff --git a/experiment-yolo_amd/ultralytics/hip/engine.py b/experiment-yolo_amd/ultralytics/hip/engine.py
--- a/experiment-yolo_amd/ultralytics/hip/engine.py
+++ b/experiment-yolo_amd/ultralytics/hip/engine.py
@@ -831,7 +831,7 @@
                 ykey = (id(y.st), y.c0, y.C)
                 rows = self._rows_grad.get(ykey)
                 if rows is not None and self._gw.get(ykey) == 1:
-                    asg, A, a0 = rows
+                    asg, A, a0 = rows[:3]
                     self.call("dy_bn_act_bwd_reduce_rows", y.gptr, y.ld, raw.ptr, raw.ld, spec.coef.data_ptr(), self._acc_ready(spec.acc_b),
                               y.N, y.H * y.W, spec.cout, spec.act, asg, A, a0)
                 else:
@@ -888,12 +888,15 @@
                 self.call("dy_copy_slice", y.gptr, y.ld, res.gptr, res.ld, npix, res.C)
         ykey = (id(y.st), y.c0, y.C)
         rows = self._rows_grad.get(ykey)
+        sparse = rows is not None and rows[3]
+        if sparse and (self._gw.get(ykey) != 1 or res is not None or not spec.trainable):
+            raise RuntimeError(f"{spec.name}: its output gradient was written at foreground rows only, but this backward would read it densely")
         if rows is not None and self._gw.get(ykey) != 1:
             rows = None
         if acc and (fused_red or reduced):
             pass
         elif acc and rows is not None and rg == (0, 0, 0):
-            asg, A, a0 = rows
+            asg, A, a0 = rows[:3]
             self.call("dy_bn_act_bwd_reduce_rows", y.gptr, y.ld, raw.ptr, raw.ld, spec.coef.data_ptr(), self._acc_ready(spec.acc_b),
                       y.N, y.H * y.W, spec.cout, spec.act, asg, A, a0)
         elif acc:
@@ -916,6 +919,8 @@
         side_small = bool(not frozen and SIDE_SMALL and npix <= SIDE_SMALL and self.deferred_wgrad is not None and not self.cur_sid and not self.side_wgrad
                           and acc and isinstance(x, Act) and x.needs_grad and spec.ld is None)
         bn_wgrad = bool(not frozen and acc and BN_WGRAD and spec.act == DY_ACT_SILU and not self.side_wgrad and not side_small and raw.ld == spec.cout)
+        if sparse and not (bn_wgrad and acc and (fused_red or reduced or rg == (0, 0, 0)) and isinstance(x, Act)):
+            raise RuntimeError(f"{spec.name}: its output gradient was written at foreground rows only, but this backward would read it densely")
         if bn_wgrad and self._wgrad_dgrad_ok(spec, x):
             draw = None
         elif ((self.side_wgrad or side_small) and self.deferred_wgrad is not None) or self.cur_sid:
@@ -925,7 +930,7 @@
             draw = self.scratch("draw", npix * spec.cout * 2)
         if bn_wgrad:
             bn = (raw, draw, spec.coef.data_ptr(), spec.acc_b.data_ptr(), spec.gbn_w.data_ptr(), spec.gbn_b.data_ptr(), float(npix))
-            self._conv_bwd(spec, x, y.gptr, y.ld, y.H, y.W, bn=bn)
+            self._conv_bwd(spec, x, y.gptr, y.ld, y.H, y.W, bn=bn, rows=rows[:3] if sparse else None)
             return
         if acc:
             self.call("dy_bn_act_bwd_apply_acc", y.gptr, y.ld, raw.ptr, raw.ld, draw.data_ptr(), spec.cout, spec.coef.data_ptr(),
@@ -959,7 +964,9 @@
         return bool(self.L.dy_conv1x1_wgrad_dgrad_supported(x.N, x.H, x.W, spec.cin, spec.cout))
 
     def _conv_bwd(self, spec, x, dy_ptr, lddy, Ho, Wo, accumulate_w=0, defer=True, bn=None, bias_acc=None, planes=None, side_hint=False,
-                  wgrad=True):
+                  wgrad=True, rows=None):
+        if rows is not None:
+            assert wgrad and bn is not None and bn[1] is not None and planes is None and spec.ld is None and isinstance(x, Act), spec.name
         if not wgrad:
             assert bn is None and bias_acc is None and planes is None
             return self._input_grad(spec, x, dy_ptr, lddy, Ho, Wo)
@@ -1021,6 +1028,8 @@
             if spec.ld is not None:
                 n, cphys, cin = spec.ld
                 self.call("dy_conv_wgrad_ld_bn", *head, spec.cout, cin, n, cphys, accumulate_w)
+            elif rows is not None:
+                self.call("dy_conv_wgrad_bn_rows", *head, spec.cin, spec.cout, spec.ks, spec.stride, accumulate_w, *rows)
             else:
                 self.call("dy_conv_wgrad_bn", *head, spec.cin, spec.cout, spec.ks, spec.stride, accumulate_w)
             dy_ptr, lddy = draw.data_ptr(), spec.cout
@@ -1173,6 +1182,11 @@
             self.pending_decode.append((spec, x, l))
         self.tape.append(lambda: self._rows_bwd_levels(items, dy_ptr_fns))
 
+    def _rows_sparse_ok(self, spec, raw):
+        return bool(os.environ.get("DY_HEAD_ROWS_SPARSE", "1") != "0" and spec.trainable and BN_WGRAD and spec.acc_b is not None
+                    and spec.act == DY_ACT_SILU and not self.side_wgrad and not SIDE_SMALL and not self.cur_sid and spec.ks == 3
+                    and spec.stride == 1 and spec.ld is None and raw.ld == spec.cout and spec.cout % 16 == 0)
+
     def _rows_bwd_levels(self, items, fns):
         if not (self.loss_rows is not None and self.deferred_wgrad is not None and not self.side_wgrad):
             for (spec, x, l), fn in zip(items, fns):
@@ -1189,7 +1203,10 @@
             self.deferred_wgrad.append((spec, slabs, ns, spec.acc_bias))
             acc = x.grad_target() if x.needs_grad else 0
             if x.needs_grad and not acc and self._sole_consumer_of_conv(x) is not None:
-                self._rows_grad[(id(x.st), x.c0, x.C)] = (asg, A, a0[l])
+                sparse = self._rows_sparse_ok(*self._sole_consumer_of_conv(x))
+                self._rows_grad[(id(x.st), x.c0, x.C)] = (asg, A, a0[l], sparse)
+                if sparse:
+                    acc = 2
             xp, xld, xc = self._src(x)
             for k, v in zip(cols, (xp, xld, xc, dyp, ld, a0[l], spec.weight.data_ptr(), x.gptr if x.needs_grad else 0, x.ld, acc,
                                    slabs.data_ptr(), self._acc_ready(spec.acc_bias), Ho, Wo)):
@@ -1257,7 +1274,7 @@
             self.deferred_wgrad.append((spec, slabs, ns, spec.acc_bias))
             acc = x.grad_target() if x.needs_grad else 0
             if x.needs_grad and not acc and self._sole_consumer_of_conv(x) is not None:
-                self._rows_grad[(id(x.st), x.c0, x.C)] = (asg, A, a0[rows_level])
+                self._rows_grad[(id(x.st), x.c0, x.C)] = (asg, A, a0[rows_level], False)
             src = self.unapplied(x)
             xp, xld, xcoef = (x.ptr, x.ld, 0) if src is None else (src[0].ptr, src[0].ld, src[1].coef.data_ptr())
             self.call("dy_conv1x1_rows_backward", xp, xld, xcoef, dyp, ld, asg, A, a0[rows_level], spec.weight.data_ptr(),
diff --git a/experiment-yolo_amd/ultralytics/hip/train.py b/experiment-yolo_amd/ultralytics/hip/train.py
--- a/experiment-yolo_amd/ultralytics/hip/train.py
+++ b/experiment-yolo_amd/ultralytics/hip/train.py
@@ -642,9 +642,9 @@
             own = int(args[8]) * int(args[9]) * e * 3
         elif name == "dy_bn_act_bwd_apply_acc":
             own = int(args[10]) * int(args[11]) * e * 3
-        elif name in ("dy_conv_wgrad_bn", "dy_conv_wgrad_ld_bn"):
+        elif name in ("dy_conv_wgrad_bn", "dy_conv_wgrad_bn_rows", "dy_conv_wgrad_ld_bn"):
             n, h, w = args[14:17]
-            if name == "dy_conv_wgrad_bn":
+            if name != "dy_conv_wgrad_ld_bn":
                 cin, cout, ks, stride = args[17:21]
             else:
                 cout, ks, stride = args[17], 1, 1
@@ -726,9 +726,9 @@
         if name == "dy_stem_wgrad_bn":
             n, h, w = args[11:14]
             return "stem_wgrad_bn_kernel", n * h * w * 3 * 2 + n * ((h - 1) // 2 + 1) * ((w - 1) // 2 + 1) * 16 * 2
-        if name in ("dy_conv_wgrad_bn", "dy_conv_wgrad_ld_bn"):
+        if name in ("dy_conv_wgrad_bn", "dy_conv_wgrad_bn_rows", "dy_conv_wgrad_ld_bn"):
             n, h, w = args[14:17]
-            if name == "dy_conv_wgrad_bn":
+            if name != "dy_conv_wgrad_ld_bn":
                 cin, cout, ks, stride = args[17:21]
             else:
                 cout, _ld_cin, ld_taps, ld_cphys = args[17:21]
@@ -736,7 +736,7 @@
             if L.dy_wgrad_kernel_name_at(n, h, w, cin, cout, ks, stride, buf, 128) == 0:
                 pad = ks // 2
                 Ho, Wo = (h + 2 * pad - ks) // stride + 1, (w + 2 * pad - ks) // stride + 1
-                return (buf.value.decode().replace(", 0>", ", 1>"),
+                return (buf.value.decode().replace(", 0>", ", 17>" if name == "dy_conv_wgrad_bn_rows" else ", 1>"),
                         n * h * w * ((cin + 7) // 8 * 8) * 2 + n * Ho * Wo * ((cout + 7) // 8 * 8) * 2)
         if name == "dy_conv_wgrad_ld":
             n, h, w, cout, ld_cin, ld_taps, ld_cphys = args[6:13]
diff --git a/include/dealyolo_hip.h b/include/dealyolo_hip.h
--- a/include/dealyolo_hip.h
+++ b/include/dealyolo_hip.h
@@ -71,6 +71,9 @@
 int dy_conv_wgrad_bn(const void* x, int ldx, const void* dy, int lddy, const void* raw, int ldraw, void* draw, const float* coef,
                      const double* acc, float* dgamma, float* dbeta, float count, float* slabs, float* dw, int n, int h, int w,
                      int cin, int cout, int ks, int stride, int accumulate, hipStream_t stream);
+int dy_conv_wgrad_bn_rows(const void* x, int ldx, const void* dy, int lddy, const void* raw, int ldraw, void* draw, const float* coef,
+                          const double* acc, float* dgamma, float* dbeta, float count, float* slabs, float* dw, int n, int h, int w,
+                          int cin, int cout, int ks, int stride, int accumulate, const int* assigned, int A, int a0, hipStream_t stream);
 int dy_conv_wgrad_ld_bn(const void* x, int ldx, const void* dy, int lddy, const void* raw, int ldraw, void* draw,
                         const float* coef, const double* acc, float* dgamma, float* dbeta, float count, float* slabs, float* dw,
                         int n, int h, int w, int cout, int ld_cin, int ld_taps, int ld_cphys, int accumulate, hipStream_t stream);
```
